# HKUST-Aerial-Robotics/FIESTA

Hardware: NVIDIA H100
Metric: esdf_voxel_updates_per_s (higher is better)
Workload: dtype int32+f64

## Files before the change

### fiesta_b200/csrc/fb_exact.cu

```cuda
#include <cub/cub.cuh>
#include <stdio.h>
#include <stdlib.h>
#include <algorithm>
#include <chrono>
#include "fb_common.cuh"
#include "fb_exact.h"

#define XNONE 0xffffffffu
#define XMB_NONE 0xffffffffffffffffull

__device__ __forceinline__ void x_coords(const FbGeom &g, uint32_t ii, int &x, int &y, int &z) {
  z = ii % (unsigned)g.pz; const unsigned xy = ii / (unsigned)g.pz; y = xy % (unsigned)g.gy; x = xy / (unsigned)g.gy;
}
__device__ __forceinline__ unsigned x_d2(int x, int y, int z, uint32_t c) {
  int ox, oy, oz; fb_unpack(c, ox, oy, oz); ox -= x; oy -= y; oz -= z;
  return (unsigned)(ox * ox + oy * oy + oz * oz);
}
__device__ __forceinline__ unsigned x_dist_of(int x, int y, int z, uint32_t c) { return c < 2u ? 0xffffffffu : x_d2(x, y, z, c); }

__global__ void k_x_flag_exist(const uint32_t *list, unsigned n, const double *occ, double l_occ, uint8_t *flags, int want) {
  const unsigned i = blockIdx.x * blockDim.x + threadIdx.x;
  if (i < n) flags[i] = ((occ[list[i]] > l_occ) ? 1 : 0) == want;
}
__global__ void k_x_apply_seed(FbGeom g, const uint32_t *E, unsigned n, uint32_t *cobs, unsigned long long *LS, unsigned long long t0) {
  const unsigned i = blockIdx.x * blockDim.x + threadIdx.x;
  if (i >= n) return;
  const uint32_t ii = E[i];
  int x, y, z; x_coords(g, ii, x, y, z);
  cobs[ii] = fb_pack(x, y, z);
  LS[ii] = t0 + i;
}

__global__ void k_x_del_minpos(const uint32_t *del, unsigned n, const double *occ, double l_occ, uint32_t *scratch) {
  const unsigned i = blockIdx.x * blockDim.x + threadIdx.x;
  if (i < n && !(occ[del[i]] > l_occ)) atomicMin(&scratch[del[i]], i);
}
__global__ void k_x_del_flag(const uint32_t *del, unsigned n, const double *occ, double l_occ, const uint32_t *scratch, uint8_t *flags) {
  const unsigned i = blockIdx.x * blockDim.x + threadIdx.x;
  if (i < n) flags[i] = (!(occ[del[i]] > l_occ) && scratch[del[i]] == i) ? 1 : 0;
}
__global__ void k_x_del_rank(const uint32_t *sel, unsigned n, uint32_t *scratch) {
  const unsigned i = blockIdx.x * blockDim.x + threadIdx.x;
  if (i < n) scratch[sel[i]] = i;
}
__global__ void k_x_scan_deps(FbGeom g, const uint32_t *cobs, const uint32_t *occbits, const uint32_t *rank, const unsigned long long *LS,
                              unsigned long long *k1, unsigned long long *k2, uint32_t *dv, unsigned *ndep, unsigned cap, int shift) {
  for (long long v = (long long)blockIdx.x * blockDim.x + threadIdx.x; v < g.ptotal; v += (long long)gridDim.x * blockDim.x) {
    const uint32_t c = cobs[v] & FB_CODE_MASK;
    bool dep = false;
    unsigned r = 0;
    if (c >= 2u) {
      int ox, oy, oz; fb_unpack(c, ox, oy, oz);
      const long long oi = fb_ii(g, ox, oy, oz);
      if (!((__ldg(&occbits[oi >> 5]) >> (oi & 31)) & 1u)) { r = rank[oi]; dep = r != XNONE; }
    }
    const unsigned slot = fb_warp_append(ndep, dep);
    if (dep && slot < cap) {
      const unsigned long long inv = ~LS[v];
      if (shift) k1[slot] = ((unsigned long long)r << shift) | (inv & ((1ull << shift) - 1ull));
      else { k1[slot] = r; k2[slot] = inv; }
      dv[slot] = (uint32_t)v;
    }
  }
}
__global__ void k_x_unset(const uint32_t *list, unsigned n, uint32_t *scratch) {
  const unsigned i = blockIdx.x * blockDim.x + threadIdx.x;
  if (i < n) scratch[list[i]] = XNONE;
}
__global__ void k_x_iota(uint32_t *a, unsigned n) { const unsigned i = blockIdx.x * blockDim.x + threadIdx.x; if (i < n) a[i] = i; }
__global__ void k_x_gather64(const unsigned long long *src, const uint32_t *idx, unsigned n, unsigned long long *dst) {
  const unsigned i = blockIdx.x * blockDim.x + threadIdx.x; if (i < n) dst[i] = src[idx[i]];
}
__global__ void k_x_gather32(const uint32_t *src, const uint32_t *idx, unsigned n, uint32_t *dst) {
  const unsigned i = blockIdx.x * blockDim.x + threadIdx.x; if (i < n) dst[i] = src[idx[i]];
}
__global__ void k_x_set_ord(const uint32_t *deps, unsigned n, uint32_t *ord, uint32_t *nc, uint8_t *nk) {
  const unsigned i = blockIdx.x * blockDim.x + threadIdx.x;
  if (i < n) { ord[deps[i]] = i; nc[i] = FB_INF; nk[i] = 24; }
}
__global__ void k_x_fill32(uint32_t *a, size_t n, uint32_t val) {
  for (size_t i = (size_t)blockIdx.x * blockDim.x + threadIdx.x; i < n; i += (size_t)gridDim.x * blockDim.x) a[i] = val;
}
__global__ void k_x_fill64(unsigned long long *a, size_t n, unsigned long long val) {
  for (size_t i = (size_t)blockIdx.x * blockDim.x + threadIdx.x; i < n; i += (size_t)gridDim.x * blockDim.x) a[i] = val;
}

static inline unsigned nblk(size_t n, unsigned t = 256) { return (unsigned)((n + t - 1) / t); }

static int x_select(FbExact *X, const uint32_t *in, const uint8_t *flags, uint32_t *out, unsigned n, unsigned *count, cudaStream_t s) {
  *count = 0;
  if (n == 0) return FIESTA_OK;
  size_t bytes = 0;
  CK(cub::DeviceSelect::Flagged(nullptr, bytes, in, flags, out, X->d_count.p, (int)n, s));
  CK(X->cub_tmp.grow(bytes, s));
  CK(cub::DeviceSelect::Flagged(X->cub_tmp.p, bytes, in, flags, out, X->d_count.p, (int)n, s));
  CK(cudaMemcpyAsync(X->h_count, X->d_count, 4, cudaMemcpyDeviceToHost, s));
  CK(cudaStreamSynchronize(s));
  *count = *X->h_count;
  return FIESTA_OK;
}
static int x_sort_pairs(FbExact *X, const unsigned long long *kin, unsigned long long *kout, const uint32_t *vin, uint32_t *vout, unsigned n, cudaStream_t s,
                        int key_bits = 64) {
  size_t bytes = 0;
  CK(cub::DeviceRadixSort::SortPairs(nullptr, bytes, kin, kout, vin, vout, (int)n, 0, key_bits, s));
  CK(X->cub_tmp.grow(bytes, s));
  CK(cub::DeviceRadixSort::SortPairs(X->cub_tmp.p, bytes, kin, kout, vin, vout, (int)n, 0, key_bits, s));
  return FIESTA_OK;
}
int fb_exact_init(FbExact *X, const FbGeom &g, int device, cudaStream_t s) {
  const size_t P = (size_t)g.ptotal;
  CK(fb_xrelax_init());
  X->relax_blocks = fb_xrelax_blocks(device);
  if (X->relax_blocks <= 0 || X->relax_blocks > FB_X_MAX_BLOCKS) { fb_set_error("exact mode init: k_x_relax does not fit on this device"); return FIESTA_ERR_CUDA; }
  CK(X->MB.alloc(P)); CK(X->LS.alloc(P)); CK(X->tkey.alloc(P));
  CK(X->touched.alloc(P));
  CK(X->SUM.alloc(P)); CK(X->SUMg.alloc(P)); CK(cudaMemsetAsync(X->SUMg, 0, P * 4, s));
  CK(X->emask.alloc(P));
  CK(X->wstamp.alloc(P)); CK(cudaMemsetAsync(X->wstamp, 0, P * 4, s));
  for (int k = 0; k < 3; ++k) { CK(X->W[k].alloc(P)); CK(X->F[k].alloc(P)); CK(cudaMemsetAsync(X->W[k], 0, P * 4, s)); }
  for (int k = 0; k < 2; ++k) CK(X->E[k].alloc(P));
  X->dense_min = 16384u;
  if (const char *e = getenv("FIESTA_X_DENSE")) { long v = atol(e); if (v >= 0 && v <= (1 << 24)) X->dense_min = (unsigned)v; }
  if (const char *e = getenv("FIESTA_X_ASYNC")) X->async = atol(e) != 0;
  if (const char *e = getenv("FIESTA_X_SMALL_ASYNC")) X->small_async = atol(e) != 0;
  X->small_max = FB_X_SMALL_DEFAULT;
  if (const char *e = getenv("FIESTA_X_SMALL")) { long v = atol(e); if (v >= 0 && v <= 65536) X->small_max = (unsigned)v; }
  CK(X->slotc.alloc(((size_t)X->small_max + 1) * 32));
  const size_t c0 = P / 8 > (1u << 20) ? P / 8 : (1u << 20);
  for (FbDevBuf<unsigned long long> *b : {&X->k1, &X->k2, &X->k1b, &X->k2b}) CK(b->grow(c0, s));
  for (FbDevBuf<uint32_t> *b : {&X->dv, &X->idx[0], &X->idx[1], &X->deps, &X->nc[0], &X->nc[1], &X->sel}) CK(b->grow(c0, s));
  CK(X->flags.grow(c0, s)); CK(X->flags2.grow(c0, s));
  CK(X->cub_tmp.grow(c0 * 16 + (64u << 20), s));
  CK(X->d_ctl.alloc(1)); CK(cudaMemsetAsync(X->d_ctl, 0, sizeof(FbXCtl), s));
  CK(X->h_ctl.alloc(1));
  CK(X->d_count.alloc(4)); CK(X->d_flag.alloc(4));
  CK(X->h_count.alloc(4));
  CK(cudaMemsetAsync(X->d_count, 0, 16, s)); CK(cudaMemsetAsync(X->d_flag, 0, 16, s));
  k_x_fill64<<<FB_SMS * 8, 256, 0, s>>>(X->MB, P, XMB_NONE);
  CK(cudaMemsetAsync(X->tkey, 0, P * 8, s));
  CK(cudaMemsetAsync(X->LS, 0, P * 8, s));
  X->tclock = 1; X->key_base = 0; X->key_epoch = 1; X->key_hi = 1ull << FB_KEY_BITS; X->gen_id = 0; X->wclock = 0; X->sclock = 0;
  CK(cudaGetLastError());
  return FIESTA_OK;
}

int fb_exact_queue_crossings(FbExact *X, const unsigned long long *ins_key, const uint32_t *ins_vox, const unsigned long long *del_key,
                             const uint32_t *del_vox, FbDevBuf<uint32_t> &ins, unsigned *n_ins, FbDevBuf<uint32_t> &del, unsigned *n_del,
                             cudaStream_t s, int *launches) {
  int r;
  CK(cudaMemcpyAsync(X->h_count, X->d_count, 8, cudaMemcpyDeviceToHost, s));
  CK(cudaStreamSynchronize(s));
  const unsigned ni = X->h_count[0], nd = X->h_count[1];
  CK(ins.grow((size_t)*n_ins + ni, s, *n_ins));
  CK(del.grow((size_t)*n_del + nd, s, *n_del));
  CK(X->k1b.grow(ni > nd ? ni : nd, s));
  if (ni) { if ((r = x_sort_pairs(X, ins_key, X->k1b, ins_vox, ins + *n_ins, ni, s, FB_KEY_BITS))) return r; *n_ins += ni; *launches += 1; }
  if (nd) { if ((r = x_sort_pairs(X, del_key, X->k1b, del_vox, del + *n_del, nd, s, FB_KEY_BITS))) return r; *n_del += nd; *launches += 1; }
  return FIESTA_OK;
}
int fb_exact_next_epoch(FbExact *X, const FbGeom &g, cudaStream_t s) {
  X->key_base = 0;
  if (++X->key_epoch >= (1u << (64 - FB_KEY_BITS))) {
    CK(cudaMemsetAsync(X->tkey, 0, (size_t)g.ptotal * 8, s));
    X->key_epoch = 1;
  }
  X->key_hi = (unsigned long long)X->key_epoch << FB_KEY_BITS;
  return FIESTA_OK;
}

int fb_exact_update_esdf(FbExact *X, const FbGeom &g, uint32_t *cobs, uint32_t *scratch, const double *occ, const uint32_t *occbits, double l_occ,
                         const uint32_t *ins, unsigned n_ins, const uint32_t *del, unsigned n_del, cudaStream_t s, FbExactStats *st, int *launches) {
  int r;
  const size_t P = (size_t)g.ptotal;
  memset(st, 0, sizeof(*st));
  CK(X->flags.grow((size_t)(n_ins > n_del ? n_ins : n_del) + 16, s));
  static const bool xdbg = getenv("FIESTA_DEBUG_X") != nullptr;
  auto now = [] { return std::chrono::steady_clock::now(); };
  auto ms = [](std::chrono::steady_clock::time_point a, std::chrono::steady_clock::time_point b) { return std::chrono::duration<double, std::milli>(b - a).count(); };
  const auto t_begin = now();
  unsigned nE = 0, ndep_run = 0;
  unsigned long long ls_deps = 0;
  bool scratch_ok = X->scratch_clean;
  if (n_ins) {
    k_x_flag_exist<<<nblk(n_ins), 256, 0, s>>>(ins, n_ins, occ, l_occ, X->flags, 1);
    if ((r = x_select(X, ins, X->flags, X->E[0], n_ins, &nE, s))) return r;
    if (nE) k_x_apply_seed<<<nblk(nE), 256, 0, s>>>(g, X->E[0], nE, cobs, X->LS, X->tclock);
    X->tclock += nE;
    *launches += 2;
  }
  if (n_del) {
    CK(X->sel.grow((size_t)n_del + 16, s));
    if (!X->scratch_clean) { k_x_fill32<<<FB_SMS * 8, 256, 0, s>>>(scratch, P, XNONE); *launches += 1; }
    scratch_ok = true;
    X->scratch_clean = false;
    k_x_del_minpos<<<nblk(n_del), 256, 0, s>>>(del, n_del, occ, l_occ, scratch);
    k_x_del_flag<<<nblk(n_del), 256, 0, s>>>(del, n_del, occ, l_occ, scratch, X->flags);
    unsigned nd = 0;
    if ((r = x_select(X, del, X->flags, X->sel, n_del, &nd, s))) return r;
    k_x_unset<<<nblk(n_del), 256, 0, s>>>(del, n_del, scratch);
    *launches += 3;
    if (nd) {
      k_x_del_rank<<<nblk(nd), 256, 0, s>>>(X->sel, nd, scratch);
      int rank_bits = 1; while ((1ull << rank_bits) < (unsigned long long)nd) ++rank_bits;
      int clock_bits = 1; while (clock_bits < 64 && (X->tclock >> clock_bits)) ++clock_bits;
      const bool two_sorts = getenv("FIESTA_X_TWO_SORTS") != nullptr;
      const int shift = (rank_bits + clock_bits <= 64 && !two_sorts) ? 64 - rank_bits : 0;
      unsigned ndep = 0;
      for (int attempt = 0; attempt < 2; ++attempt) {
        const size_t cap = std::min({X->dv.cap, X->k1.cap, X->k2.cap});
        CK(cudaMemsetAsync(X->d_count, 0, 4, s));
        k_x_scan_deps<<<FB_SMS * 16, 256, 0, s>>>(g, cobs, occbits, scratch, X->LS, X->k1, X->k2, X->dv, X->d_count, (unsigned)cap, shift);
        CK(cudaMemcpyAsync(X->h_count, X->d_count, 4, cudaMemcpyDeviceToHost, s));
        CK(cudaStreamSynchronize(s));
        ndep = *X->h_count;
        *launches += 1;
        if (ndep <= cap) break;
        CK(X->dv.grow(ndep, s));
        CK(X->k1.grow(ndep, s));
        CK(X->k2.grow(ndep, s));
      }
      st->dependants = ndep;
      k_x_unset<<<nblk(nd), 256, 0, s>>>(X->sel, nd, scratch);
      if (ndep) {
        CK(X->k1b.grow(ndep, s));
        CK(X->k2b.grow(ndep, s));
        CK(X->idx[0].grow(ndep, s));
        CK(X->idx[1].grow(ndep, s));
        CK(X->deps.grow(ndep, s));
        CK(X->nc[0].grow(ndep, s));
        CK(X->nc[1].grow(ndep, s));
        CK(X->flags.grow(ndep, s));
        if (shift) {
          if ((r = x_sort_pairs(X, X->k1, X->k1b, X->dv, X->deps, ndep, s))) return r;
          *launches += 1;
        } else {
          k_x_iota<<<nblk(ndep), 256, 0, s>>>(X->idx[0], ndep);
          if ((r = x_sort_pairs(X, X->k2, X->k2b, X->idx[0], X->idx[1], ndep, s))) return r;
          k_x_gather64<<<nblk(ndep), 256, 0, s>>>(X->k1, X->idx[1], ndep, X->k1b);
          if ((r = x_sort_pairs(X, X->k1b, X->k2b, X->idx[1], X->idx[0], ndep, s))) return r;
          k_x_gather32<<<nblk(ndep), 256, 0, s>>>(X->dv, X->idx[0], ndep, X->deps);
          *launches += 5;
        }
        CK(X->flags2.grow(ndep, s));
        k_x_set_ord<<<nblk(ndep), 256, 0, s>>>(X->deps, ndep, scratch, X->nc[0], X->flags2);
        *launches += 1;
        ndep_run = ndep; ls_deps = X->tclock;
        X->tclock += ndep;
      }
    }
  }
  st->generations = 0;
  if (xdbg) { cudaStreamSynchronize(s); fprintf(stderr, "[x] seeds+deletes %.2f ms (reseed rounds %u, dependants %u)\n", ms(t_begin, now()), st->reseed_rounds, st->dependants); }
  if (nE || ndep_run) {
    if (xdbg && !X->d_dbg) CK(X->d_dbg.alloc(FB_X_DBG_WORDS));
    if (xdbg) CK(cudaMemsetAsync(X->d_dbg, 0, FB_X_DBG_WORDS * 8, s));
    if (X->sclock > 0xf0000000u) { CK(cudaMemsetAsync(X->SUMg, 0, P * 4, s)); X->sclock = 0; }
    if (X->gen_id > 0xf0000000u) X->gen_id = 0;
    if (X->wclock > 0xf0000000u) { CK(cudaMemsetAsync(X->wstamp, 0, P * 4, s)); X->wclock = 0; }
    FbXCtl *h = X->h_ctl;
    memset(h, 0, sizeof(*h));
    h->gen_id = X->gen_id; h->wclock = X->wclock; h->tclock = X->tclock; h->sclock = X->sclock;
    CK(cudaMemcpyAsync(X->d_ctl, h, sizeof(FbXCtl), cudaMemcpyHostToDevice, s));
    CK(fb_xrelax_launch(X, g, cobs, nE, X->deps, ndep_run, scratch, X->nc[0], X->flags2, occbits, ls_deps, xdbg ? X->d_dbg.p : nullptr, s));
    if (ndep_run) k_x_unset<<<nblk(ndep_run), 256, 0, s>>>(X->deps, ndep_run, scratch);
    CK(cudaMemcpyAsync(h, X->d_ctl, sizeof(FbXCtl), cudaMemcpyDeviceToHost, s));
    CK(cudaStreamSynchronize(s));
    *launches += 1;
    if (h->err) {
      if (h->err == 3u) {
        for (int k = 0; k < 3; ++k) CK(cudaMemsetAsync(X->W[k], 0, P * 4, s));
        CK(cudaMemsetAsync(X->wstamp, 0, P * 4, s));
        X->wclock = 0;
      }
      fb_set_error(h->err == 1u ? "exact mode: generation with more than 2^27 entries"
                   : h->err == 3u ? "exact mode: a wait of the asynchronous work queue exceeded its bound" : "exact mode: behaviour fixpoint did not converge");
      return FIESTA_ERR_CUDA;
    }
    X->gen_id = h->gen_id; X->wclock = h->wclock; X->tclock = h->tclock; X->sclock = h->sclock;
    st->generations = h->generations; st->reseed_rounds = h->reseed_rounds; st->eval_rounds = h->rounds; st->dense_rounds = h->dense_rounds;
    st->voxels_changed = h->voxels_changed; st->expansions = h->expansions;
    if (xdbg) {
      static unsigned long long hd[FB_X_DBG_WORDS];
      static double cyc_per_us = 0;
      if (cyc_per_us == 0) { int dev = 0, khz = 0; CK(cudaGetDevice(&dev)); CK(cudaDeviceGetAttribute(&khz, cudaDevAttrClockRate, dev)); cyc_per_us = khz / 1000.0; }
      CK(cudaMemcpy(hd, X->d_dbg, sizeof(hd), cudaMemcpyDeviceToHost));
      static const char *cat[20] = {"S", "round1", "rounds", "dense", "commit", "apply", "s.round1", "s.rounds", "s.commit", "s.apply", "top", "empty-barrier",
                                    "reseed.rounds", "reseed.assemble", "", "", "async", "", "refresh", "s.async"};
      fprintf(stderr, "[x] reseed rounds %u; phases (us, count):", st->reseed_rounds);
      for (int c = 0; c < 20; ++c)
        if (*cat[c]) fprintf(stderr, " %s %.0f/%llu", cat[c], hd[FB_XDBG_PHASE + 2 * c] / cyc_per_us, hd[FB_XDBG_PHASE + 2 * c + 1]);
      fprintf(stderr, "\n");
      fprintf(stderr, "[x] round work (summed longest CTA work time us / summed list length):");
      for (int c : {1, 2, 3, 6, 7}) fprintf(stderr, " %s %.0f/%llu", cat[c], hd[FB_XDBG_WORK + 2 * c] / cyc_per_us, hd[FB_XDBG_WORK + 2 * c + 1]);
      fprintf(stderr, "\n");
      for (int h = 0; h < 2; ++h) {
        fprintf(stderr, "[x] list-length histogram %s (log2 bucket=rounds):", h ? "s.rounds" : "rounds");
        for (int b = 0; b < 32; ++b) if (hd[FB_XDBG_NWH + 32 * h + b]) fprintf(stderr, " %d=%llu", b, hd[FB_XDBG_NWH + 32 * h + b]);
        fprintf(stderr, "\n");
      }
      fprintf(stderr, "[x] async: evaluations %llu dirty %llu pushes %llu spin %.0f us\n", hd[FB_XDBG_Q + 0], hd[FB_XDBG_Q + 1], hd[FB_XDBG_Q + 2],
              hd[FB_XDBG_Q + 3] / cyc_per_us);
      for (int gq = 0; gq < 2; ++gq) { fprintf(stderr, "[x] gen %d work lists:", gq); for (int r = 0; r < 512 && hd[FB_XDBG_ROUNDS + gq * 512 + r]; ++r) fprintf(stderr, " %llu", hd[FB_XDBG_ROUNDS + gq * 512 + r]); fprintf(stderr, "\n"); }
      fprintf(stderr, "[x] work-list entries: evaluated %llu refreshed %llu reseeded %llu\n", hd[FB_XDBG_PHASE + 2 * 14], hd[FB_XDBG_PHASE + 2 * 14 + 1], hd[FB_XDBG_PHASE + 2 * 15]);
      fprintf(stderr, "[x] gens %u rounds %u dense %u deps %u nE0 %u |", st->generations, st->eval_rounds, st->dense_rounds, st->dependants, nE);
      for (unsigned q = 0; q < st->generations && q < FB_XDBG_GENS; ++q) fprintf(stderr, " %llu/%llu/%.1fus", hd[3 * q], hd[3 * q + 1], hd[3 * q + 2] / cyc_per_us);
      fprintf(stderr, "\n");
    }
  }
  X->scratch_clean = scratch_ok;
  return FIESTA_OK;
}
```

### fiesta_b200/csrc/fb_exact.h

```cpp
#pragma once
#include "fb_common.cuh"

#define FB_X_MAX_BLOCKS 256
#define FB_X_SMALL_DEFAULT 32768u
#define FB_XDBG_GENS 1024
#define FB_XDBG_NCAT 24
#define FB_XDBG_NQ 8
#define FB_XDBG_PHASE (3 * FB_XDBG_GENS)
#define FB_XDBG_ROUNDS (FB_XDBG_PHASE + 2 * FB_XDBG_NCAT)
#define FB_XDBG_WMAX (FB_XDBG_ROUNDS + 2 * 512)
#define FB_XDBG_WORK (FB_XDBG_WMAX + 4096)
#define FB_XDBG_NWH (FB_XDBG_WORK + 2 * FB_XDBG_NCAT)
#define FB_XDBG_Q (FB_XDBG_NWH + 2 * 32)
#define FB_X_DBG_WORDS (FB_XDBG_Q + FB_XDBG_NQ)

struct FbExactStats {
  unsigned long long expansions;
  unsigned long long voxels_changed;
  unsigned generations, eval_rounds, dense_rounds, reseed_rounds, dependants;
};

struct FbXCtl {
  unsigned bar, err;
  unsigned sclock, pad1;
  unsigned nW[3], nF[3];
  unsigned gen_id, wclock;
  unsigned generations, rounds, dense_rounds, reseed_rounds;
  unsigned long long tclock, expansions, voxels_changed;
  unsigned partial[FB_X_MAX_BLOCKS];
  alignas(128) unsigned long long qtail;
  alignas(128) unsigned qhead;
  alignas(128) unsigned qdone;
};

struct FbExact {
  FbDevBuf<unsigned long long> MB;
  FbDevBuf<unsigned long long> LS;
  FbDevBuf<unsigned long long> tkey;
  FbDevBuf<uint32_t> touched;
  unsigned long long tclock = 0;
  unsigned long long key_base = 0;
  unsigned long long key_hi = 0;
  unsigned key_epoch = 0;
  FbDevBuf<unsigned> d_count, d_flag;
  FbHostBuf<unsigned> h_count;
  bool scratch_clean = false;
  FbDevBuf<uint4> SUM;
  FbDevBuf<uint32_t> SUMg;
  unsigned gen_id = 0, wclock = 0, sclock = 0;
  FbDevBuf<uint32_t> emask;
  FbDevBuf<uint32_t> W[3], F[3];
  FbDevBuf<uint32_t> wstamp;
  FbDevBuf<uint32_t> slotc;
  unsigned dense_min = 0;
  unsigned small_max = 0;
  bool async = true;
  bool small_async = false;
  FbDevBuf<FbXCtl> d_ctl;
  FbHostBuf<FbXCtl> h_ctl;
  FbDevBuf<unsigned long long> d_dbg;
  int relax_blocks = 0;
  FbDevBuf<uint32_t> E[2], sel;
  FbDevBuf<unsigned long long> k1, k2, k1b, k2b;
  FbDevBuf<uint32_t> dv, idx[2], deps, nc[2];
  FbDevBuf<uint8_t> flags, flags2;
  FbDevBuf<char> cub_tmp;
};

int fb_exact_init(FbExact *X, const FbGeom &g, int device, cudaStream_t s);
int fb_exact_queue_crossings(FbExact *X, const unsigned long long *ins_key, const uint32_t *ins_vox, const unsigned long long *del_key,
                             const uint32_t *del_vox, FbDevBuf<uint32_t> &ins, unsigned *n_ins, FbDevBuf<uint32_t> &del, unsigned *n_del,
                             cudaStream_t s, int *launches);
int fb_exact_next_epoch(FbExact *X, const FbGeom &g, cudaStream_t s);
int fb_exact_update_esdf(FbExact *X, const FbGeom &g, uint32_t *cobs, uint32_t *scratch, const double *occ, const uint32_t *occbits, double l_occ,
                         const uint32_t *ins, unsigned n_ins, const uint32_t *del, unsigned n_del, cudaStream_t s, FbExactStats *st, int *launches);
cudaError_t fb_xrelax_init();
int fb_xrelax_blocks(int device);
cudaError_t fb_xrelax_launch(FbExact *X, const FbGeom &g, uint32_t *cobs, unsigned nE0, const uint32_t *deps, unsigned ndep, uint32_t *ord, uint32_t *nc, uint8_t *nk,
                             const uint32_t *occbits, unsigned long long ls_deps, unsigned long long *dbg, cudaStream_t s);
```

### fiesta_b200/csrc/fb_xrelax.cu

```cuda
#include <stdio.h>
#include "fb_common.cuh"
#include "fb_exact.h"
#include "fb_divmagic.h"

#define XT 1024
#define XW (XT / 32)
#define XNONE 0xffffffffu
#define X_DEAD 0ull
#define X_PULL 1ull
#define X_PUSH 2ull
#define XMB_NONE 0xffffffffffffffffull
#define X_NOFF 129
#define X_MAX_ROUNDS 4000000u
#define XGB 8
#define XRC 8
#define XDBG_PHASE FB_XDBG_PHASE
#define XDBG_ROUNDS FB_XDBG_ROUNDS
#define XDBG_WMAX FB_XDBG_WMAX

static __constant__ int x_dirs[24][3] = {
    {-1, 0, 0}, {1, 0, 0}, {0, -1, 0}, {0, 1, 0}, {0, 0, -1}, {0, 0, 1},
    {-1, -1, 0}, {1, 1, 0}, {0, -1, -1}, {0, 1, 1}, {-1, 0, -1}, {1, 0, 1},
    {-1, 1, 0}, {1, -1, 0}, {0, -1, 1}, {0, 1, -1}, {1, 0, -1}, {-1, 0, 1},
    {-2, 0, 0}, {2, 0, 0}, {0, -2, 0}, {0, 2, 0}, {0, 0, -2}, {0, 0, 2}};
static __constant__ int x_off_c[X_NOFF];

__device__ __forceinline__ unsigned x_vi(const FbGeom &g, int x, int y, int z) { return (unsigned)((x * g.gy + y) * g.pz + z); }
__device__ __forceinline__ bool x_in_grid(const FbGeom &g, int x, int y, int z) {
  return (unsigned)x < (unsigned)g.gx && (unsigned)y < (unsigned)g.gy && (unsigned)z < (unsigned)g.gz;
}
__device__ __forceinline__ bool x_in_range(const FbGeom &g, int x, int y, int z) {
  return (unsigned)(x - g.min_vec[0]) <= (unsigned)(g.max_vec[0] - g.min_vec[0]) && (unsigned)(y - g.min_vec[1]) <= (unsigned)(g.max_vec[1] - g.min_vec[1]) &&
         (unsigned)(z - g.min_vec[2]) <= (unsigned)(g.max_vec[2] - g.min_vec[2]);
}
__device__ __forceinline__ int x_dc(int j, int k) {
  const int D[24][3] = {{-1, 0, 0}, {1, 0, 0}, {0, -1, 0}, {0, 1, 0}, {0, 0, -1}, {0, 0, 1}, {-1, -1, 0}, {1, 1, 0}, {0, -1, -1}, {0, 1, 1}, {-1, 0, -1}, {1, 0, 1},
                        {-1, 1, 0}, {1, -1, 0}, {0, -1, 1}, {0, 1, -1}, {1, 0, -1}, {-1, 0, 1}, {-2, 0, 0}, {2, 0, 0}, {0, -2, 0}, {0, 2, 0}, {0, 0, -2}, {0, 0, 2}};
  return D[j][k];
}
__device__ __forceinline__ unsigned long long x_writer_word(const FbGeom &g, const unsigned long long *MB, unsigned v, int x, int y, int z, int j, bool inr) {
  const int dx = x_dc(j, 0), dy = x_dc(j, 1), dz = x_dc(j, 2);
  const bool ok = inr && (dx == 0 || (unsigned)(x - dx) < (unsigned)g.gx) && (dy == 0 || (unsigned)(y - dy) < (unsigned)g.gy) &&
                  (dz == 0 || (unsigned)(z - dz) < (unsigned)g.gz);
  return ok ? __ldcg(&MB[v - (unsigned)((dx * g.gy + dy) * g.pz + dz)]) : XMB_NONE;
}

struct XShared {
  int off[X_NOFF];
  int dir[32];
  unsigned char slot[25 * 24];
  unsigned char self[32];
  unsigned red[XW], red2[XW];
  unsigned base, total;
  unsigned qdone;
};

__device__ __forceinline__ unsigned x_d2(int x, int y, int z, uint32_t c) {
  int ox, oy, oz; fb_unpack(c, ox, oy, oz); ox -= x; oy -= y; oz -= z;
  return (unsigned)(ox * ox + oy * oy + oz * oz);
}
__device__ __forceinline__ unsigned x_dist_of(int x, int y, int z, uint32_t c) { return c < 2u ? 0xffffffffu : x_d2(x, y, z, c); }
__device__ __forceinline__ unsigned long long x_mb(unsigned par, unsigned i, unsigned long long kind, uint32_t code) {
  return ((unsigned long long)(par & 1u) << 63) | ((unsigned long long)i << 33) | (kind << 31) | (unsigned long long)(code & FB_CODE_MASK);
}
__device__ __forceinline__ unsigned x_mb_idx(unsigned long long w) { return (unsigned)(w >> 33) & 0x7ffffffu; }
__device__ __forceinline__ unsigned x_mb_par(unsigned long long w) { return (unsigned)(w >> 63); }
__device__ __forceinline__ unsigned long long x_mb_kind(unsigned long long w) { return (w >> 31) & 3ull; }
__device__ __forceinline__ uint32_t x_mb_code(unsigned long long w) { return (uint32_t)(w & FB_CODE_MASK); }

struct XState { unsigned d; uint32_t c; unsigned ts; };
struct XNb { unsigned long long w[X_NOFF + 3]; uint32_t c[28]; };

template <bool WANT_FIRST>
__device__ __forceinline__ XState x_gather(const FbGeom &g, const uint32_t *cobs, const unsigned long long *MB, int x, int y, int z, unsigned T,
                                           unsigned &first, uint32_t &snap) {
  XState s;
  const unsigned v = x_vi(g, x, y, z);
  const bool inr = x_in_range(g, x, y, z);
  unsigned long long w[XGB];
  const uint32_t snap_raw = __ldcg(&cobs[v]);
  const unsigned long long wown = __ldcg(&MB[v]);
#pragma unroll
  for (int j = 0; j < XGB; ++j) w[j] = x_writer_word(g, MB, v, x, y, z, j, inr);
  snap = snap_raw & FB_CODE_MASK;
  s.c = snap; s.d = (snap_raw & FB_DINF) ? 0xffffffffu : x_dist_of(x, y, z, s.c); s.ts = XNONE;
  first = XNONE;
  const unsigned d0 = s.d;
  if (s.c == FB_UNKNOWN) return s;
#pragma unroll
  for (int h = 0; h < 24 / XGB; ++h) {
    if (h >= 1) {
#pragma unroll
      for (int j = 0; j < XGB; ++j) w[j] = x_writer_word(g, MB, v, x, y, z, XGB * h + j, inr);
    }
#pragma unroll
    for (int j = 0; j < XGB; ++j) {
      const unsigned long long ww = w[j];
      if (ww == XMB_NONE || x_mb_kind(ww) != X_PUSH) continue;
      const unsigned ts = x_mb_idx(ww) * 32u + (unsigned)(XGB * h + j);
      const uint32_t c = x_mb_code(ww);
      const unsigned d = x_d2(x, y, z, c);
      if (d < d0) {
        if (WANT_FIRST && ts < first) first = ts;
        if (ts < T && (d < s.d || (d == s.d && ts < s.ts))) { s.d = d; s.c = c; s.ts = ts; }
      }
    }
  }
  if (wown != XMB_NONE && x_mb_kind(wown) == X_PULL) {
    const unsigned ts = x_mb_idx(wown) * 32u + 24u;
    const uint32_t c = x_mb_code(wown);
    const unsigned d = x_d2(x, y, z, c);
    if (d < d0) {
      if (WANT_FIRST && ts < first) first = ts;
      if (ts < T && (d < s.d || (d == s.d && ts < s.ts))) { s.d = d; s.c = c; s.ts = ts; }
    }
  }
  return s;
}
__device__ __forceinline__ void x_summarize(const FbGeom &g, const uint32_t *cobs, const unsigned long long *MB, uint4 *SUM, int x, int y, int z) {
  unsigned first; uint32_t snap;
  const XState f = x_gather<true>(g, cobs, MB, x, y, z, XNONE, first, snap);
  SUM[x_vi(g, x, y, z)] = make_uint4(first, f.ts, f.c, snap);
}
template <bool USE_SUM>
__device__ __forceinline__ XState x_state(const FbGeom &g, const uint32_t *cobs, const unsigned long long *MB, const uint4 *SUM, int x, int y, int z,
                                          unsigned T, uint32_t &snap) {
  unsigned first;
  if (USE_SUM) {
    const uint4 u = __ldcg(&SUM[x_vi(g, x, y, z)]);
    snap = u.w;
    XState s;
    if (u.x == XNONE || T <= u.x) { s.c = u.w; s.d = x_dist_of(x, y, z, s.c); s.ts = XNONE; return s; }
    if (T > u.y) { s.c = u.z; s.d = x_dist_of(x, y, z, s.c); s.ts = u.y; return s; }
  }
  return x_gather<false>(g, cobs, MB, x, y, z, T, first, snap);
}

__device__ __forceinline__ unsigned x_ld_acquire(const unsigned *p) {
  unsigned v;
  asm volatile("ld.acquire.gpu.global.u32 %0, [%1];" : "=r"(v) : "l"(p) : "memory");
  return v;
}
__device__ __forceinline__ void x_gsync(unsigned *bar, unsigned &target) {
  __syncthreads();
  if (threadIdx.x == 0) {
    target += gridDim.x;
    asm volatile("red.release.gpu.global.add.u32 [%0], %1;" ::"l"(bar), "r"(1u) : "memory");
    while (x_ld_acquire(bar) < target) { }
  }
  __syncthreads();
}

struct XArgs {
  FbGeom g;
  uint32_t *cobs;
  unsigned long long *MB, *LS;
  uint4 *SUM;
  uint32_t *SUMg;
  uint32_t *E[2];
  uint32_t *emask;
  uint32_t *W[3], *F[3];
  uint32_t *wstamp;
  uint32_t *slotc;
  FbXCtl *ctl;
  unsigned nE0, small_max, dense_min;
  const uint32_t *deps; unsigned ndep;
  uint32_t *ord;
  uint32_t *nc;
  uint8_t *nk;
  const uint32_t *occbits;
  unsigned long long ls_deps;
  unsigned long long *dbg;
  unsigned div_pz_m, div_pz_s, div_gy_m, div_gy_s;
  unsigned async_on;
  unsigned small_async_on;
};
__device__ __forceinline__ unsigned x_div(unsigned n, unsigned m, unsigned s) { return m ? (__umulhi(n, m) >> s) : n; }
__device__ __forceinline__ void x_coords(const XArgs &a, uint32_t ii, int &x, int &y, int &z) {
  const unsigned xy = x_div(ii, a.div_pz_m, a.div_pz_s);
  z = (int)(ii - xy * (unsigned)a.g.pz);
  const unsigned xx = x_div(xy, a.div_gy_m, a.div_gy_s);
  y = (int)(xy - xx * (unsigned)a.g.gy);
  x = (int)xx;
}

__device__ __forceinline__ void x_unpack_off(int o, int &dx, int &dy, int &dz) { dx = (o & 15) - 4; dy = ((o >> 4) & 15) - 4; dz = ((o >> 8) & 15) - 4; }

__device__ __forceinline__ void x_claim_summaries(const XArgs &a, const XShared &sh, unsigned lane, int x, int y, int z, unsigned sclock) {
  if (lane >= 25u) return;
  int dx, dy, dz; x_unpack_off(sh.dir[lane], dx, dy, dz);
  const int nx = x + dx, ny = y + dy, nz = z + dz;
  if (!x_in_grid(a.g, nx, ny, nz) || !(lane == 24u || x_in_range(a.g, nx, ny, nz))) return;
  const unsigned n = x_vi(a.g, nx, ny, nz);
  if (__ldcg(&a.SUMg[n]) != sclock && atomicExch(&a.SUMg[n], sclock) != sclock) x_summarize(a.g, a.cobs, a.MB, a.SUM, nx, ny, nz);
}

__device__ __forceinline__ void x_refresh_summaries(const XArgs &a, const XShared &sh, unsigned lane, unsigned i, uint32_t p, int x, int y, int z) {
  unsigned long long w = 0;
  if (lane == 0) w = __ldcg(&a.MB[p]);
  w = __shfl_sync(0xffffffffu, w, 0);
  if (lane >= 25u) return;
  int dx, dy, dz; x_unpack_off(sh.dir[lane], dx, dy, dz);
  const int nx = x + dx, ny = y + dy, nz = z + dz;
  if (!x_in_grid(a.g, nx, ny, nz) || !(lane == 24u || x_in_range(a.g, nx, ny, nz))) return;
  const uint4 u = __ldcg(&a.SUM[x_vi(a.g, nx, ny, nz)]);
  if (u.w == FB_UNKNOWN) return;
  const unsigned ts = i * 32u + lane;
  bool redo = u.x == ts || u.y == ts;
  if (!redo) {
    const unsigned long long kind = x_mb_kind(w);
    const uint32_t c = x_mb_code(w);
    if (((kind == X_PUSH && lane < 24u) || (kind == X_PULL && lane == 24u)) && c >= 2u) {
      const unsigned d = x_d2(nx, ny, nz, c);
      if (u.y == XNONE) redo = true;
      else { const unsigned bd = x_d2(nx, ny, nz, u.z); redo = ts < u.x || d < bd || (d == bd && ts < u.y); }
    }
  }
  if (redo) x_summarize(a.g, a.cobs, a.MB, a.SUM, nx, ny, nz);
}

__device__ __forceinline__ void x_list_affected(const XArgs &a, const XShared &sh, unsigned lane, unsigned i, int x, int y, int z, unsigned nof,
                                                unsigned wclock, unsigned out) {
  const FbGeom &g = a.g;
  unsigned long long w[5];
#pragma unroll
  for (int t = 0; t < 5; ++t) {
    const unsigned o = lane + 32u * (unsigned)t;
    w[t] = XMB_NONE;
    if (o < nof) {
      int dx, dy, dz; x_unpack_off(sh.off[o], dx, dy, dz);
      const int nx = x + dx, ny = y + dy, nz = z + dz;
      if (x_in_grid(g, nx, ny, nz)) w[t] = __ldcg(&a.MB[x_vi(g, nx, ny, nz)]);
    }
  }
  unsigned j[5], st[5];
#pragma unroll
  for (int t = 0; t < 5; ++t) {
    j[t] = w[t] != XMB_NONE ? x_mb_idx(w[t]) : 0u;
    st[t] = (w[t] != XMB_NONE && j[t] > i) ? __ldcg(&a.wstamp[j[t]]) : wclock;
  }
  unsigned pm = 0;
#pragma unroll
  for (int t = 0; t < 5; ++t)
    if (st[t] != wclock && atomicExch(&a.wstamp[j[t]], wclock) != wclock) pm |= 1u << t;
  const unsigned cnt = (unsigned)__popc(pm);
  unsigned incl = cnt;
#pragma unroll
  for (int o = 1; o < 32; o <<= 1) { const unsigned v = __shfl_up_sync(0xffffffffu, incl, o); if ((int)lane >= o) incl += v; }
  const unsigned total = __shfl_sync(0xffffffffu, incl, 31);
  if (total == 0u) return;
  unsigned base = 0;
  if (lane == 0) base = atomicAdd(&a.ctl->nW[out], total);
  base = __shfl_sync(0xffffffffu, base, 0) + incl - cnt;
#pragma unroll
  for (int t = 0; t < 5; ++t) if ((pm >> t) & 1u) a.W[out][base++] = j[t];
}

template <bool USE_SUM>
__device__ __forceinline__ unsigned long long x_eval(const XArgs &a, const XShared &sh, unsigned lane, unsigned par, unsigned i, uint32_t p, int x, int y, int z) {
  const FbGeom &g = a.g;
  const unsigned T0 = i * 32u;
  int qx = x, qy = y, qz = z;
  bool valid = lane == 24;
  if (lane < 24) {
    int dx, dy, dz; x_unpack_off(sh.dir[lane], dx, dy, dz);
    qx += dx; qy += dy; qz += dz;
    valid = x_in_range(g, qx, qy, qz) && x_in_grid(g, qx, qy, qz);
  }
  XState st; st.d = 0xffffffffu; st.c = 0; st.ts = XNONE;
  uint32_t snap = 0;
  if (valid) st = x_state<USE_SUM>(g, a.cobs, a.MB, a.SUM, qx, qy, qz, T0, snap);
  const unsigned sd = __shfl_sync(0xffffffffu, st.d, 24);
  const uint32_t sc = __shfl_sync(0xffffffffu, st.c, 24);
  const uint32_t c0 = __shfl_sync(0xffffffffu, snap, 24);
  if (sd != x_dist_of(x, y, z, c0)) return x_mb(par, i, X_DEAD, 0);
  unsigned long long key = ~0ull;
  if (lane < 24 && valid && st.c >= 2u) {
    const unsigned t = x_d2(x, y, z, st.c);
    if (t < sd) key = ((unsigned long long)t << 8) | lane;
  }
  unsigned long long best = key;
#pragma unroll
  for (int o = 16; o > 0; o >>= 1) { const unsigned long long other = __shfl_xor_sync(0xffffffffu, best, o); best = other < best ? other : best; }
  if (best == ~0ull) return x_mb(par, i, X_PUSH, sc);
  return x_mb(par, i, X_PULL, __shfl_sync(0xffffffffu, st.c, (int)(best & 0xffu)));
}

__device__ __forceinline__ void x_stage(const XArgs &a, const XShared &sh, XNb &nb, unsigned lane, int x, int y, int z) {
  const FbGeom &g = a.g;
  unsigned long long w[5];
#pragma unroll
  for (int t = 0; t < 5; ++t) {
    const unsigned o = lane + 32u * (unsigned)t;
    w[t] = XMB_NONE;
    if (o < X_NOFF) {
      int dx, dy, dz; x_unpack_off(sh.off[o], dx, dy, dz);
      const int nx = x + dx, ny = y + dy, nz = z + dz;
      if (x_in_grid(g, nx, ny, nz)) w[t] = __ldcg(&a.MB[x_vi(g, nx, ny, nz)]);
    }
  }
  uint32_t c = 0;
  if (lane < 25u) {
    int dx, dy, dz; x_unpack_off(sh.dir[lane], dx, dy, dz);
    const int nx = x + dx, ny = y + dy, nz = z + dz;
    if (x_in_grid(g, nx, ny, nz)) c = __ldcg(&a.cobs[x_vi(g, nx, ny, nz)]);
  }
  __syncwarp();
#pragma unroll
  for (int t = 0; t < 5; ++t) { const unsigned o = lane + 32u * (unsigned)t; if (o < X_NOFF) nb.w[o] = w[t]; }
  if (lane < 25u) nb.c[lane] = c;
  __syncwarp();
}
__device__ __forceinline__ XState x_state_nb(const FbGeom &g, const XShared &sh, const XNb &nb, unsigned lane, int qx, int qy, int qz, unsigned T, uint32_t &snap) {
  XState s;
  const uint32_t raw = nb.c[lane];
  snap = raw & FB_CODE_MASK;
  s.c = snap; s.d = (raw & FB_DINF) ? 0xffffffffu : x_dist_of(qx, qy, qz, snap); s.ts = XNONE;
  const unsigned d0 = s.d;
  if (snap == FB_UNKNOWN) return s;
  if (x_in_range(g, qx, qy, qz)) {
#pragma unroll 8
    for (int k = 0; k < 24; ++k) {
      const unsigned long long ww = nb.w[sh.slot[lane * 24u + (unsigned)k]];
      if (ww == XMB_NONE || x_mb_kind(ww) != X_PUSH) continue;
      const unsigned ts = x_mb_idx(ww) * 32u + (unsigned)k;
      const uint32_t c = x_mb_code(ww);
      const unsigned d = x_d2(qx, qy, qz, c);
      if (d < d0 && ts < T && (d < s.d || (d == s.d && ts < s.ts))) { s.d = d; s.c = c; s.ts = ts; }
    }
  }
  const unsigned long long wown = nb.w[sh.self[lane]];
  if (wown != XMB_NONE && x_mb_kind(wown) == X_PULL) {
    const unsigned ts = x_mb_idx(wown) * 32u + 24u;
    const uint32_t c = x_mb_code(wown);
    const unsigned d = x_d2(qx, qy, qz, c);
    if (d < d0 && ts < T && (d < s.d || (d == s.d && ts < s.ts))) { s.d = d; s.c = c; s.ts = ts; }
  }
  return s;
}
__device__ __forceinline__ unsigned long long x_eval_nb(const XArgs &a, const XShared &sh, const XNb &nb, unsigned lane, unsigned par, unsigned i, int x, int y, int z) {
  const FbGeom &g = a.g;
  const unsigned T0 = i * 32u;
  int qx = x, qy = y, qz = z;
  bool valid = lane == 24;
  if (lane < 24) {
    int dx, dy, dz; x_unpack_off(sh.dir[lane], dx, dy, dz);
    qx += dx; qy += dy; qz += dz;
    valid = x_in_range(g, qx, qy, qz) && x_in_grid(g, qx, qy, qz);
  }
  XState st; st.d = 0xffffffffu; st.c = 0; st.ts = XNONE;
  uint32_t snap = 0;
  if (valid) st = x_state_nb(g, sh, nb, lane, qx, qy, qz, T0, snap);
  const unsigned sd = __shfl_sync(0xffffffffu, st.d, 24);
  const uint32_t sc = __shfl_sync(0xffffffffu, st.c, 24);
  const uint32_t c0 = __shfl_sync(0xffffffffu, snap, 24);
  if (sd != x_dist_of(x, y, z, c0)) return x_mb(par, i, X_DEAD, 0);
  unsigned long long key = ~0ull;
  if (lane < 24 && valid && st.c >= 2u) {
    const unsigned t = x_d2(x, y, z, st.c);
    if (t < sd) key = ((unsigned long long)t << 8) | lane;
  }
  unsigned long long best = key;
#pragma unroll
  for (int o = 16; o > 0; o >>= 1) { const unsigned long long other = __shfl_xor_sync(0xffffffffu, best, o); best = other < best ? other : best; }
  if (best == ~0ull) return x_mb(par, i, X_PUSH, sc);
  return x_mb(par, i, X_PULL, __shfl_sync(0xffffffffu, st.c, (int)(best & 0xffu)));
}
__device__ __forceinline__ void x_list_affected_nb(const XArgs &a, const XNb &nb, unsigned lane, unsigned i, unsigned nof, unsigned wclock, unsigned out) {
  unsigned j[5], st[5];
#pragma unroll
  for (int t = 0; t < 5; ++t) {
    const unsigned o = lane + 32u * (unsigned)t;
    const unsigned long long w = o < nof ? nb.w[o] : XMB_NONE;
    j[t] = w != XMB_NONE ? x_mb_idx(w) : 0u;
    st[t] = (w != XMB_NONE && j[t] > i) ? __ldcg(&a.wstamp[j[t]]) : wclock;
  }
  unsigned pm = 0;
#pragma unroll
  for (int t = 0; t < 5; ++t)
    if (st[t] != wclock && atomicExch(&a.wstamp[j[t]], wclock) != wclock) pm |= 1u << t;
  const unsigned cnt = (unsigned)__popc(pm);
  unsigned incl = cnt;
#pragma unroll
  for (int o = 1; o < 32; o <<= 1) { const unsigned v = __shfl_up_sync(0xffffffffu, incl, o); if ((int)lane >= o) incl += v; }
  const unsigned total = __shfl_sync(0xffffffffu, incl, 31);
  if (total == 0u) return;
  unsigned base = 0;
  if (lane == 0) base = atomicAdd(&a.ctl->nW[out], total);
  base = __shfl_sync(0xffffffffu, base, 0) + incl - cnt;
#pragma unroll
  for (int t = 0; t < 5; ++t) if ((pm >> t) & 1u) a.W[out][base++] = j[t];
}

__device__ __forceinline__ unsigned x_block_scan(XShared &sh, unsigned c, unsigned lane, unsigned wid, unsigned &total) {
  unsigned incl = c;
#pragma unroll
  for (int o = 1; o < 32; o <<= 1) { const unsigned t = __shfl_up_sync(0xffffffffu, incl, o); if ((int)lane >= o) incl += t; }
  __syncthreads();
  if (lane == 31) sh.red[wid] = incl;
  __syncthreads();
  const unsigned v = sh.red[lane]; unsigned s = v;
#pragma unroll
  for (int o = 1; o < 32; o <<= 1) { const unsigned t = __shfl_up_sync(0xffffffffu, s, o); if ((int)lane >= o) s += t; }
  total = __shfl_sync(0xffffffffu, s, 31);
  return __shfl_sync(0xffffffffu, s - v, (int)wid) + incl - c;
}

__device__ __forceinline__ unsigned x_warp_append_n(unsigned *counter, unsigned n, unsigned lane) {
  const unsigned act = __activemask(), below = (1u << lane) - 1u;
  unsigned pre = 0, total = 0;
#pragma unroll
  for (int bit = 0; bit < 4; ++bit) {
    const unsigned m = __ballot_sync(act, (n >> bit) & 1u);
    pre += (unsigned)__popc(m & below) << bit;
    total += (unsigned)__popc(m) << bit;
  }
  if (total == 0u) return 0u;
  const int leader = __ffs(act) - 1;
  unsigned base = 0;
  if ((int)lane == leader) base = atomicAdd(counter, total);
  return __shfl_sync(act, base, leader) + pre;
}

#define X_Q_FULL 0x80000000u
#define X_Q_WAIT_NS 2000000000ull
__device__ __forceinline__ unsigned x_ld_relaxed(const unsigned *p) {
  unsigned v;
  asm volatile("ld.relaxed.gpu.global.u32 %0, [%1];" : "=r"(v) : "l"(p) : "memory");
  return v;
}
__device__ __forceinline__ unsigned long long x_globaltimer() {
  unsigned long long t;
  asm volatile("mov.u64 %0, %%globaltimer;" : "=l"(t));
  return t;
}
__device__ __forceinline__ void x_q_abort(const XArgs &a) {
  atomicCAS(&a.ctl->err, 0u, 3u);
  atomicExch(&a.ctl->qdone, 1u);
}
__device__ __forceinline__ unsigned x_q_count(const XArgs &a, XShared &sh, unsigned long long delta) {
  const unsigned long long old = atomicAdd(&a.ctl->qtail, delta);
  if ((unsigned)((old + delta) >> 32) == 0u) { atomicExch(&a.ctl->qdone, 1u); sh.qdone = 1u; }
  return (unsigned)old;
}
__device__ __forceinline__ void x_q_put(const XArgs &a, XShared &sh, uint32_t *ring, unsigned cap, unsigned idx, unsigned e) {
  unsigned *slot = &ring[idx % cap];
  const volatile unsigned *done = &sh.qdone;
  unsigned cur = x_ld_relaxed(slot);
  const unsigned long long t0 = x_globaltimer();
  for (unsigned it = 0;; ++it) {
    if (!(cur & X_Q_FULL)) {
      const unsigned o = atomicCAS(slot, cur, e | X_Q_FULL);
      if (o == cur) return;
      cur = o;
      continue;
    }
    if (*done) return;
    if ((it & 15u) == 15u) {
      if (x_ld_acquire(&a.ctl->qdone)) { sh.qdone = 1u; return; }
      if (x_globaltimer() - t0 > X_Q_WAIT_NS) { x_q_abort(a); sh.qdone = 1u; return; }
    }
    __nanosleep(64);
    cur = x_ld_relaxed(slot);
  }
}
template <bool DBG>
__device__ __forceinline__ unsigned x_q_take(const XArgs &a, XShared &sh, uint32_t *ring, unsigned cap, unsigned &h) {
  if (h == XNONE) h = atomicAdd(&a.ctl->qhead, 1u);
  unsigned *slot = &ring[h % cap];
  const volatile unsigned *done = &sh.qdone;
  const long long c0 = DBG ? clock64() : 0;
  unsigned long long t0 = 0;
  unsigned ns = 32;
  for (unsigned it = 0;; ++it) {
    if (x_ld_relaxed(slot) & X_Q_FULL) {
      const unsigned v = atomicExch(slot, 0u);
      if (v & X_Q_FULL) { h = XNONE; if (DBG) atomicAdd(&a.dbg[FB_XDBG_Q + 3], (unsigned long long)(clock64() - c0)); return v & ~X_Q_FULL; }
    }
    if (*done) break;
    if ((it & 15u) == 15u) {
      if (x_ld_acquire(&a.ctl->qdone)) { sh.qdone = 1u; break; }
      const unsigned long long t = x_globaltimer();
      if (t0 == 0) t0 = t;
      else if (t - t0 > X_Q_WAIT_NS) { x_q_abort(a); sh.qdone = 1u; break; }
    }
    __nanosleep(ns);
    ns = ns < 256u ? 2u * ns : 256u;
  }
  if (DBG) atomicAdd(&a.dbg[FB_XDBG_Q + 3], (unsigned long long)(clock64() - c0));
  return XNONE;
}
__device__ __forceinline__ unsigned x_q_list(const XArgs &a, XShared &sh, const XNb &nb, uint32_t *ring, unsigned cap, unsigned lane, unsigned i, unsigned nof, unsigned A) {
  unsigned j[5], st[5];
#pragma unroll
  for (int t = 0; t < 5; ++t) {
    const unsigned o = lane + 32u * (unsigned)t;
    const unsigned long long w = o < nof ? nb.w[o] : XMB_NONE;
    j[t] = w != XMB_NONE ? x_mb_idx(w) : 0u;
    st[t] = (w != XMB_NONE && j[t] > i) ? x_ld_relaxed(&a.wstamp[j[t]]) : A + 1u;
  }
  unsigned pm = 0;
#pragma unroll
  for (int t = 0; t < 5; ++t)
    if (st[t] != A + 1u && atomicMax(&a.wstamp[j[t]], A + 1u) < A) pm |= 1u << t;
  const unsigned cnt = (unsigned)__popc(pm);
  unsigned incl = cnt;
#pragma unroll
  for (int o = 1; o < 32; o <<= 1) { const unsigned v = __shfl_up_sync(0xffffffffu, incl, o); if ((int)lane >= o) incl += v; }
  const unsigned total = __shfl_sync(0xffffffffu, incl, 31);
  if (total == 0u) return 0u;
  unsigned base = 0;
  if (lane == 0) base = x_q_count(a, sh, (unsigned long long)total * 0x100000001ull);
  base = __shfl_sync(0xffffffffu, base, 0) + incl - cnt;
#pragma unroll
  for (int t = 0; t < 5; ++t) if ((pm >> t) & 1u) x_q_put(a, sh, ring, cap, base++, j[t]);
  return total;
}
template <bool BIG, bool DBG>
__device__ __forceinline__ void x_q_run(const XArgs &a, XShared &sh, XNb &stg, unsigned lane, const uint32_t *E, unsigned nE, uint32_t *ring,
                                        unsigned gen, unsigned A, unsigned fout, unsigned i, bool claimed) {
  const uint32_t p = __ldcg(&E[i]);
  int x, y, z; x_coords(a, p, x, y, z);
  for (;; claimed = false) {
    if (DBG && lane == 0) atomicAdd(&a.dbg[FB_XDBG_Q + 0], 1ull);
    if (!claimed) {
      if (lane == 0) atomicExch(&a.wstamp[i], A);
      __syncwarp();
      __threadfence();
    }
    x_stage(a, sh, stg, lane, x, y, z);
    const unsigned long long old = stg.w[0], nw2 = x_eval_nb(a, sh, stg, lane, gen, i, x, y, z);
    if (nw2 != old) {
      if (lane == 0) {
        a.MB[p] = nw2;
        if (BIG) {
          const unsigned f = atomicAdd(&a.ctl->nF[fout], 1u);
          if (f < (unsigned)a.g.ptotal) a.F[fout][f] = i;
        }
      }
      __syncwarp();
      __threadfence();
      const unsigned np = x_q_list(a, sh, stg, ring, nE, lane, i, (x_mb_kind(old) == X_PUSH || x_mb_kind(nw2) == X_PUSH) ? (unsigned)X_NOFF : 25u, A);
      if (DBG && lane == 0 && np) atomicAdd(&a.dbg[FB_XDBG_Q + 2], (unsigned long long)np);
    }
    unsigned again = 0;
    if (lane == 0) again = atomicCAS(&a.wstamp[i], A, A - 1u) != A ? 1u : 0u;
    if (!__shfl_sync(0xffffffffu, again, 0)) break;
    if (DBG && lane == 0) atomicAdd(&a.dbg[FB_XDBG_Q + 1], 1ull);
  }
}
template <bool DBG>
__device__ void x_async(const XArgs &a, XShared &sh, XNb &stg, unsigned lane, unsigned gwarp, unsigned gwarps, const uint32_t *E, unsigned nE,
                        const uint32_t *wl, unsigned nw, uint32_t *ring, unsigned gen, unsigned A, unsigned fout) {
  for (unsigned q0 = gwarp * 32u; q0 < nw; q0 += gwarps * 32u) {
    const unsigned q = q0 + lane;
    const unsigned e = q < nw ? __ldcg(&wl[q]) : 0u;
    const bool push = q < nw && atomicMax(&a.wstamp[e], A + 1u) < A;
    const unsigned pm = __ballot_sync(0xffffffffu, push), cnt = (unsigned)__popc(pm);
    if (cnt == 0u) continue;
    unsigned base = 0;
    if (lane == 0) base = x_q_count(a, sh, (unsigned long long)cnt * 0x100000001ull);
    base = __shfl_sync(0xffffffffu, base, 0);
    if (push) x_q_put(a, sh, ring, nE, base + (unsigned)__popc(pm & ((1u << lane) - 1u)), e);
    if (DBG && lane == 0) atomicAdd(&a.dbg[FB_XDBG_Q + 2], (unsigned long long)cnt);
  }
  if (lane == 0) x_q_count(a, sh, 0ull - (1ull << 32));
  unsigned h = XNONE;
  for (;;) {
    unsigned i = 0;
    if (lane == 0) i = x_q_take<DBG>(a, sh, ring, nE, h);
    i = __shfl_sync(0xffffffffu, i, 0);
    if (i == XNONE) break;
    x_q_run<true, DBG>(a, sh, stg, lane, E, nE, ring, gen, A, fout, i, false);
    if (lane == 0) x_q_count(a, sh, 0ull - (1ull << 32));
  }
}
template <bool DBG>
__device__ void x_async_small(const XArgs &a, XShared &sh, XNb &stg, unsigned lane, unsigned gwarp, unsigned gwarps, const uint32_t *E, unsigned nE,
                              uint32_t *ring, unsigned gen, unsigned A) {
  const unsigned nwk = min(gwarps, nE);
  if (gwarp >= nwk) return;
  if (gwarp == 0u && lane == 0 && nwk < gwarps) x_q_count(a, sh, 0ull - ((unsigned long long)(gwarps - nwk) << 32));
  for (unsigned s0 = gwarp; s0 < nE; s0 += 32u * nwk) {
    const unsigned e = s0 + lane * nwk;
    unsigned om = __ballot_sync(0xffffffffu, e < nE && atomicMax(&a.wstamp[e], A) < A);
    __threadfence();
    while (om) {
      const unsigned i = s0 + (unsigned)(__ffs(om) - 1) * nwk;
      om &= om - 1u;
      x_q_run<false, DBG>(a, sh, stg, lane, E, nE, ring, gen, A, 0u, i, true);
    }
  }
  if (lane == 0) x_q_count(a, sh, 0ull - (1ull << 32));
  unsigned h = XNONE;
  for (;;) {
    unsigned i = 0;
    if (lane == 0) i = x_q_take<DBG>(a, sh, ring, nE, h);
    i = __shfl_sync(0xffffffffu, i, 0);
    if (i == XNONE) break;
    x_q_run<false, DBG>(a, sh, stg, lane, E, nE, ring, gen, A, 0u, i, false);
    if (lane == 0) x_q_count(a, sh, 0ull - (1ull << 32));
  }
}

__device__ __forceinline__ uint32_t x_reseed_eval(const XArgs &a, unsigned i, int x, int y, int z, unsigned &kc) {
  const FbGeom &g = a.g;
  kc = 24u;
  for (int k = 0; k < 24; ++k) {
    const int nx = x + x_dirs[k][0], ny = y + x_dirs[k][1], nz = z + x_dirs[k][2];
    if (!x_in_range(g, nx, ny, nz) || !x_in_grid(g, nx, ny, nz)) continue;
    const unsigned nv = x_vi(g, nx, ny, nz);
    const unsigned o = __ldcg(&a.ord[nv]);
    uint32_t c;
    if (o != XNONE) { if (o < i) c = __ldcg(&a.nc[o]); else continue; }
    else c = __ldcg(&a.cobs[nv]) & FB_CODE_MASK;
    if (c >= 2u) {
      int ox, oy, oz; fb_unpack(c, ox, oy, oz);
      const unsigned oi = x_vi(g, ox, oy, oz);
      if ((__ldg(&a.occbits[oi >> 5]) >> (oi & 31)) & 1u) { kc = (unsigned)k; return c; }
    }
  }
  return FB_INF;
}

extern __shared__ __align__(16) unsigned char x_dyn_smem[];

template <bool DBG>
__global__ void __launch_bounds__(XT, 1) k_x_relax(const XArgs a) {
  __shared__ XShared sh;
  const FbGeom &g = a.g;
  FbXCtl *ctl = a.ctl;
  const unsigned tid = threadIdx.x, lane = tid & 31u, wid = tid >> 5;
  const unsigned G = gridDim.x, b = blockIdx.x;
  const unsigned gtid = b * XT + tid, gthreads = G * XT;
  const unsigned gwarp = gtid >> 5, gwarps = gthreads >> 5;
  for (unsigned k = tid; k < X_NOFF; k += XT) sh.off[k] = x_off_c[k];
  if (tid < 32) sh.self[tid] = 0;
  if (tid == 0) sh.qdone = 0u;
  if (gtid == 0) a.ctl->qtail = (unsigned long long)gwarps << 32;
  if (tid < 32) sh.dir[tid] = tid < 24 ? ((x_dirs[tid][0] + 4) | ((x_dirs[tid][1] + 4) << 4) | ((x_dirs[tid][2] + 4) << 8)) : (4 | (4 << 4) | (4 << 8));
  __syncthreads();
  for (unsigned q = tid; q < 25u * 24u + 25u; q += XT) {
    const unsigned t = q < 600u ? q / 24u : q - 600u, k = q < 600u ? q % 24u : 24u;
    int tx, ty, tz, kx = 0, ky = 0, kz = 0; x_unpack_off(sh.dir[t], tx, ty, tz);
    if (k < 24u) x_unpack_off(sh.dir[k], kx, ky, kz);
    const int code = (tx - kx + 4) | ((ty - ky + 4) << 4) | ((tz - kz + 4) << 8);
    unsigned found = 0;
    for (unsigned o = 0; o < X_NOFF; ++o) if (sh.off[o] == code) found = o;
    if (q < 600u) sh.slot[q] = (unsigned char)found; else sh.self[t] = (unsigned char)found;
  }
  __syncthreads();
  XNb &stg = reinterpret_cast<XNb *>(x_dyn_smem)[wid];

  unsigned nE = a.nE0, bar_target = 0;
  int cur = 0;
  unsigned gen = ctl->gen_id, wclock = ctl->wclock;
  unsigned long long tclock = ctl->tclock;
  unsigned generations = 0, rounds_total = 0, dense_total = 0;
  unsigned long long changed_total = 0;
  if (DBG) {
    const long long t0 = clock64();
    for (int q = 0; q < 32; ++q) x_gsync(&ctl->bar, bar_target);
    if (gtid == 0) a.dbg[XDBG_PHASE + 2 * 11] = (unsigned long long)(clock64() - t0) / 32ull;
  }
  long long t_ph = DBG ? clock64() : 0;
#define X_LAP(cat) do { if (DBG && gtid == 0) { const long long t_now = clock64(); a.dbg[XDBG_PHASE + 2 * (cat)] += (unsigned long long)(t_now - t_ph); a.dbg[XDBG_PHASE + 2 * (cat) + 1] += 1ull; t_ph = t_now; } } while (0)
  unsigned reseed_rounds = 0;
  if (a.ndep) {
    for (unsigned r = 1;; ++r) {
      const unsigned in = r % 3u, out = (r + 1u) % 3u, zz = (r + 2u) % 3u;
      const unsigned nw = r == 1u ? a.ndep : __ldcg(&ctl->nW[in]);
      if (gtid == 0) ctl->nW[zz] = 0;
      if (r > 1u && nw == 0u) break;
      if (DBG && gtid == 0) a.dbg[XDBG_PHASE + 2 * 15] += nw;
      ++reseed_rounds; ++wclock;
      if (nw <= 2u * gwarps) {
        for (unsigned q = gwarp; q < nw; q += gwarps) {
          const unsigned i = r == 1u ? q : __ldcg(&a.W[in][q]);
          int x, y, z; x_coords(a, __ldcg(&a.deps[i]), x, y, z);
          int dx = 0, dy = 0, dz = 0;
          if (lane < 24u) x_unpack_off(sh.dir[lane], dx, dy, dz);
          const int nx = x + dx, ny = y + dy, nz = z + dz;
          const bool ing = lane < 24u && x_in_grid(g, nx, ny, nz);
          const unsigned nv = ing ? x_vi(g, nx, ny, nz) : 0u;
          const unsigned o = ing ? __ldcg(&a.ord[nv]) : XNONE;
          uint32_t c = 0;
          if (ing && x_in_range(g, nx, ny, nz)) {
            if (o != XNONE) { if (o < i) c = __ldcg(&a.nc[o]); }
            else c = __ldcg(&a.cobs[nv]) & FB_CODE_MASK;
          }
          bool ok = false;
          if (c >= 2u) { int px, py, pz; fb_unpack(c, px, py, pz); const unsigned oi = x_vi(g, px, py, pz); ok = (__ldg(&a.occbits[oi >> 5]) >> (oi & 31)) & 1u; }
          const unsigned vm = __ballot_sync(0xffffffffu, ok);
          const unsigned kc = vm ? (unsigned)(__ffs(vm) - 1) : 24u;
          const uint32_t res = vm ? __shfl_sync(0xffffffffu, c, (int)kc) : FB_INF;
          uint32_t was = 0;
          if (lane == 0) { was = __ldcg(&a.nc[i]); a.nk[i] = (uint8_t)kc; }
          was = __shfl_sync(0xffffffffu, was, 0);
          if (res == was) continue;
          if (lane == 0) a.nc[i] = res;
          bool push = ing && o != XNONE && o > i;
          if (push) {
            const unsigned so = __ldcg(&a.wstamp[o]);
            push = so != wclock;
            if (push && r > 1u && so != wclock - 1u) {
              const unsigned ko = __ldcg(&a.nk[o]), kd = lane ^ 1u;
              push = kd == ko || (kd < ko && res >= 2u);
            }
            push = push && atomicExch(&a.wstamp[o], wclock) != wclock;
          }
          const unsigned slot2 = fb_warp_append(&ctl->nW[out], push);
          if (push) a.W[out][slot2] = o;
        }
      } else
      for (unsigned q = gtid; q < nw; q += gthreads) {
        const unsigned i = r == 1u ? q : __ldcg(&a.W[in][q]);
        int x, y, z; x_coords(a, __ldcg(&a.deps[i]), x, y, z);
        unsigned kc;
        const uint32_t res = x_reseed_eval(a, i, x, y, z, kc);
        const uint32_t was = __ldcg(&a.nc[i]);
        a.nk[i] = (uint8_t)kc;
        if (res == was) continue;
        a.nc[i] = res;
#pragma unroll
        for (int k0 = 0; k0 < 24; k0 += XRC) {
          unsigned o[XRC], so[XRC], ko[XRC];
#pragma unroll
          for (int t = 0; t < XRC; ++t) {
            const int k = k0 + t, nx = x + x_dc(k, 0), ny = y + x_dc(k, 1), nz = z + x_dc(k, 2);
            o[t] = x_in_grid(g, nx, ny, nz) ? __ldcg(&a.ord[x_vi(g, nx, ny, nz)]) : XNONE;
          }
#pragma unroll
          for (int t = 0; t < XRC; ++t) so[t] = (o[t] != XNONE && o[t] > i) ? __ldcg(&a.wstamp[o[t]]) : wclock;
#pragma unroll
          for (int t = 0; t < XRC; ++t) ko[t] = (so[t] != wclock && r > 1u && so[t] != wclock - 1u) ? __ldcg(&a.nk[o[t]]) : XNONE;
          unsigned pm = 0;
#pragma unroll
          for (int t = 0; t < XRC; ++t) {
            const unsigned kd = (unsigned)(k0 + t) ^ 1u;
            bool push = so[t] != wclock;
            if (push && ko[t] != XNONE) push = kd == ko[t] || (kd < ko[t] && res >= 2u);
            if (push && atomicExch(&a.wstamp[o[t]], wclock) != wclock) pm |= 1u << t;
          }
          unsigned slot2 = x_warp_append_n(&ctl->nW[out], (unsigned)__popc(pm), lane);
#pragma unroll
          for (int t = 0; t < XRC; ++t) if ((pm >> t) & 1u) a.W[out][slot2++] = o[t];
        }
      }
      x_gsync(&ctl->bar, bar_target);
    }
    X_LAP(12);
    const unsigned per = (a.ndep + G - 1u) / G;
    const unsigned lo = min(a.ndep, b * per), hi = min(a.ndep, lo + per);
    unsigned mine = 0;
    for (unsigned i = lo + tid; i < hi; i += XT) mine += __ldcg(&a.nc[i]) >= 2u ? 1u : 0u;
    unsigned tot;
    x_block_scan(sh, mine, lane, wid, tot);
    if (tid == 0) ctl->partial[b] = tot;
    if (gtid == 0) { ctl->nW[0] = ctl->nW[1] = ctl->nW[2] = 0; }
    x_gsync(&ctl->bar, bar_target);
    if (wid == 0) {
      unsigned before = 0, all = 0;
      for (unsigned k = lane; k < G; k += 32u) { const unsigned c = __ldcg(&ctl->partial[k]); all += c; if (k < b) before += c; }
#pragma unroll
      for (int o = 16; o > 0; o >>= 1) { before += __shfl_xor_sync(0xffffffffu, before, o); all += __shfl_xor_sync(0xffffffffu, all, o); }
      if (lane == 0) { sh.base = before; sh.total = all; }
    }
    __syncthreads();
    unsigned run = nE + sh.base;
    for (unsigned i0 = lo; i0 < hi; i0 += XT) {
      const unsigned i = i0 + tid;
      uint32_t c = FB_INF, v = 0;
      if (i < hi) {
        c = __ldcg(&a.nc[i]); v = __ldcg(&a.deps[i]);
        a.cobs[v] = c;
        a.LS[v] = a.ls_deps + i;
      }
      unsigned ctot;
      const unsigned pos = x_block_scan(sh, (i < hi && c >= 2u) ? 1u : 0u, lane, wid, ctot);
      if (i < hi && c >= 2u) a.E[0][run + pos] = v;
      run += ctot;
    }
    nE += sh.total;
    x_gsync(&ctl->bar, bar_target);
    X_LAP(13);
  }
  bool big = nE > a.small_max;

  ++gen;
  unsigned sclock = ctl->sclock;
  for (unsigned i = gtid; i < nE; i += gthreads) {
    const uint32_t v = __ldcg(&a.E[0][i]);
    a.MB[v] = x_mb(gen, i, X_PUSH, __ldcg(&a.cobs[v]) & FB_CODE_MASK);
  }
  x_gsync(&ctl->bar, bar_target);

  while (nE) {
    const long long t_gen = DBG ? clock64() : 0;
    X_LAP(10);
    ++generations;
    const uint32_t *E = a.E[cur];
    unsigned rounds = 0;
    bool aborted = false;
    if (big) {
      ++sclock;
      for (unsigned i = gwarp; i < nE; i += gwarps) { int x, y, z; x_coords(a, __ldcg(&E[i]), x, y, z); x_claim_summaries(a, sh, lane, x, y, z, sclock); }
      x_gsync(&ctl->bar, bar_target);
      X_LAP(0);
    }
    for (unsigned r = 1;; ++r) {
      const unsigned in = r % 3u, out = (r + 1u) % 3u, zz = (r + 2u) % 3u;
      const unsigned nw = r == 1u ? nE : __ldcg(&ctl->nW[in]);
      const unsigned nf = (big && r > 1u) ? __ldcg(&ctl->nF[in]) : 0u;
      if (gtid == 0) { ctl->nW[zz] = 0; ctl->nF[zz] = 0; }
      if (r > 1u && nw == 0u && nf == 0u) break;
      if (r > X_MAX_ROUNDS) { if (gtid == 0) ctl->err = 2u; break; }
      if (DBG && gtid == 0) { a.dbg[XDBG_PHASE + 2 * 14] += nw; a.dbg[XDBG_PHASE + 2 * 14 + 1] += nf; }
      if (a.async_on && (big ? r > 1u && nw <= a.dense_min : r == 1u && a.small_async_on)) {
        ++rounds; wclock += 3u;
        const unsigned A = wclock - 1u;
        if (big) x_async<DBG>(a, sh, stg, lane, gwarp, gwarps, E, nE, a.W[in], nw, a.W[out], gen, A, out);
        else x_async_small<DBG>(a, sh, stg, lane, gwarp, gwarps, E, nE, a.W[out], gen, A);
        x_gsync(&ctl->bar, bar_target);
        X_LAP(big ? 16 : 19);
        if (tid == 0) sh.qdone = 0u;
        if (gtid == 0) { ctl->qtail = (unsigned long long)gwarps << 32; ctl->qhead = 0u; ctl->qdone = 0u; }
        if (__ldcg(&ctl->err)) { aborted = true; break; }
        if (!big) break;
        const unsigned nfa = __ldcg(&ctl->nF[out]);
        if (nfa > (unsigned)g.ptotal) {
          ++sclock;
          for (unsigned i = gwarp; i < nE; i += gwarps) { int x, y, z; x_coords(a, __ldcg(&E[i]), x, y, z); x_claim_summaries(a, sh, lane, x, y, z, sclock); }
        } else {
          for (unsigned q = gwarp; q < nf + nfa; q += gwarps) {
            const unsigned i = q < nf ? __ldcg(&a.F[in][q]) : __ldcg(&a.F[out][q - nf]);
            const uint32_t p = __ldcg(&E[i]);
            int x, y, z; x_coords(a, p, x, y, z);
            x_refresh_summaries(a, sh, lane, i, p, x, y, z);
          }
        }
        x_gsync(&ctl->bar, bar_target);
        X_LAP(18);
        break;
      }
      ++rounds; ++wclock;
      const bool dense = big && r > 1u && nw > a.dense_min;
      if (dense) {
        ++dense_total;
        if (nf < nE / 4u) {
          for (unsigned q = gwarp; q < nf; q += gwarps) {
            const unsigned i = __ldcg(&a.F[in][q]);
            const uint32_t p = __ldcg(&E[i]);
            int x, y, z; x_coords(a, p, x, y, z);
            x_refresh_summaries(a, sh, lane, i, p, x, y, z);
          }
        } else {
          ++sclock;
          for (unsigned i = gwarp; i < nE; i += gwarps) { int x, y, z; x_coords(a, __ldcg(&E[i]), x, y, z); x_claim_summaries(a, sh, lane, x, y, z, sclock); }
        }
        x_gsync(&ctl->bar, bar_target);
      }
      const bool use_sum = big && (r == 1u || dense);
      const unsigned nref = (big && !dense) ? nf : 0u;
      const uint32_t *wl = a.W[in];
      const long long t_w0 = DBG ? clock64() : 0;
      for (unsigned q = gwarp; q < nw + nref; q += gwarps) {
        if (q >= nw) {
          const unsigned i = __ldcg(&a.F[in][q - nw]);
          const uint32_t p = __ldcg(&E[i]);
          int x, y, z; x_coords(a, p, x, y, z);
          x_refresh_summaries(a, sh, lane, i, p, x, y, z);
          continue;
        }
        const unsigned i = r == 1u ? q : __ldcg(&wl[q]);
        const uint32_t p = __ldcg(&E[i]);
        int x, y, z; x_coords(a, p, x, y, z);
        if (!use_sum) {
          x_stage(a, sh, stg, lane, x, y, z);
          const unsigned long long old = stg.w[0], nw2 = x_eval_nb(a, sh, stg, lane, gen, i, x, y, z);
          if (nw2 == old) continue;
          if (lane == 0) {
            a.MB[p] = nw2;
            if (big) a.F[out][atomicAdd(&ctl->nF[out], 1u)] = i;
          }
          x_list_affected_nb(a, stg, lane, i, (x_mb_kind(old) == X_PUSH || x_mb_kind(nw2) == X_PUSH) ? (unsigned)X_NOFF : 25u, wclock, out);
          continue;
        }
        unsigned long long old = 0;
        if (lane == 0) old = __ldcg(&a.MB[p]);
        const unsigned long long nb = x_eval<true>(a, sh, lane, gen, i, p, x, y, z);
        old = __shfl_sync(0xffffffffu, old, 0);
        if (nb == old) continue;
        if (lane == 0) {
          a.MB[p] = nb;
          if (big) a.F[out][atomicAdd(&ctl->nF[out], 1u)] = i;
        }
        x_list_affected(a, sh, lane, i, x, y, z, (x_mb_kind(old) == X_PUSH || x_mb_kind(nb) == X_PUSH) ? (unsigned)X_NOFF : 25u, wclock, out);
      }
      if (DBG) { __syncthreads(); if (tid == 0) atomicMax(&a.dbg[XDBG_WMAX + ((rounds_total + rounds) & 4095u)], (unsigned long long)(clock64() - t_w0)); }
      x_gsync(&ctl->bar, bar_target);
      X_LAP(big ? (r == 1u ? 1 : (dense ? 3 : 2)) : (r == 1u ? 6 : 7));
      if (DBG && gtid == 0) {
        if (generations <= 2u && rounds <= 512u) a.dbg[XDBG_ROUNDS + (generations - 1u) * 512u + (rounds - 1u)] = nw;
        const unsigned cat = big ? (r == 1u ? 1u : (dense ? 3u : 2u)) : (r == 1u ? 6u : 7u);
        unsigned long long *wm = &a.dbg[XDBG_WMAX + ((rounds_total + rounds) & 4095u)];
        a.dbg[FB_XDBG_WORK + 2 * cat] += __ldcg(wm); a.dbg[FB_XDBG_WORK + 2 * cat + 1] += nw; *wm = 0;
        if (cat == 2u || cat == 7u) a.dbg[FB_XDBG_NWH + (cat == 7u ? 32u : 0u) + (nw ? 32u - __clz(nw) : 0u)] += 1ull;
      }
    }
    rounds_total += rounds;
    if (rounds > X_MAX_ROUNDS || aborted) break;

    const unsigned per = (nE + G - 1u) / G;
    const unsigned lo = min(nE, b * per), hi = min(nE, lo + per);
    unsigned wcount = 0, wlive = 0;
    for (unsigned i = lo + wid; i < hi; i += XW) {
      const uint32_t p = __ldcg(&E[i]);
      int x, y, z; x_coords(a, p, x, y, z);
      unsigned long long w = 0;
      if (!big) { x_stage(a, sh, stg, lane, x, y, z); w = stg.w[0]; }
      else { if (lane == 0) w = __ldcg(&a.MB[p]); w = __shfl_sync(0xffffffffu, w, 0); }
      const unsigned long long kind = x_mb_kind(w);
      bool win = false;
      if ((kind == X_PUSH && lane < 24) || (kind == X_PULL && lane == 24)) {
        int dx, dy, dz; x_unpack_off(sh.dir[lane], dx, dy, dz);
        const int nx = x + dx, ny = y + dy, nz = z + dz;
        if (x_in_grid(g, nx, ny, nz) && (lane == 24 || x_in_range(g, nx, ny, nz))) {
          const unsigned ts = i * 32u + lane;
          if (big) win = __ldcg(&a.SUM[x_vi(g, nx, ny, nz)]).y == ts;
          else {
            uint32_t snap;
            const XState f = x_state_nb(g, sh, stg, lane, nx, ny, nz, XNONE, snap);
            win = f.ts == ts;
            if (win) a.slotc[ts] = f.c;
          }
        }
      }
      const unsigned m = __ballot_sync(0xffffffffu, win);
      if (lane == 0) { a.emask[i] = m; wcount += __popc(m); wlive += kind != X_DEAD ? 1u : 0u; }
    }
    if (lane == 0) { sh.red[wid] = wcount; sh.red2[wid] = wlive; }
    __syncthreads();
    if (wid == 0) {
      unsigned c = sh.red[lane], l = sh.red2[lane];
#pragma unroll
      for (int o = 16; o > 0; o >>= 1) { c += __shfl_xor_sync(0xffffffffu, c, o); l += __shfl_xor_sync(0xffffffffu, l, o); }
      if (lane == 0) { ctl->partial[b] = c; if (l) atomicAdd(&ctl->expansions, (unsigned long long)l); }
    }
    if (gtid == 0) { ctl->nW[0] = ctl->nW[1] = ctl->nW[2] = 0; ctl->nF[0] = ctl->nF[1] = ctl->nF[2] = 0; }
    x_gsync(&ctl->bar, bar_target);
    X_LAP(big ? 4 : 8);

    if (wid == 0) {
      unsigned before = 0, all = 0;
      for (unsigned k = lane; k < G; k += 32u) { const unsigned c = __ldcg(&ctl->partial[k]); all += c; if (k < b) before += c; }
#pragma unroll
      for (int o = 16; o > 0; o >>= 1) { before += __shfl_xor_sync(0xffffffffu, before, o); all += __shfl_xor_sync(0xffffffffu, all, o); }
      if (lane == 0) { sh.base = before; sh.total = all; }
    }
    __syncthreads();
    const unsigned n2 = sh.total;
    const bool big2 = n2 > a.small_max;
    uint32_t *En = a.E[cur ^ 1];
    unsigned run = sh.base;
    for (unsigned i0 = lo; i0 < hi; i0 += XT) {
      const unsigned i = i0 + tid;
      const uint32_t m = i < hi ? __ldcg(&a.emask[i]) : 0u;
      if (i < hi) {
        const uint32_t p = __ldcg(&E[i]);
        const unsigned long long w = __ldcg(&a.MB[p]);
        if (w != XMB_NONE && x_mb_par(w) == (gen & 1u)) atomicCAS(&a.MB[p], w, XMB_NONE);
      }
      unsigned ctot;
      unsigned r = run + x_block_scan(sh, (unsigned)__popc(m), lane, wid, ctot);
      if (m) {
        const uint32_t p = __ldcg(&E[i]);
        int x, y, z; x_coords(a, p, x, y, z);
        uint32_t me = m;
        while (me) {
          const int k = __ffs(me) - 1; me &= me - 1u;
          int dx, dy, dz; x_unpack_off(sh.dir[k], dx, dy, dz);
          const uint32_t v = (uint32_t)x_vi(g, x + dx, y + dy, z + dz);
          const unsigned ts = i * 32u + (unsigned)k;
          const uint32_t code = big ? __ldcg(&a.SUM[v]).z : __ldcg(&a.slotc[ts]);
          a.cobs[v] = code;
          a.LS[v] = tclock + ts;
          En[r] = v;
          a.MB[v] = x_mb(gen + 1u, r, X_PUSH, code);
          ++r;
        }
      }
      run += ctot;
    }
    if (DBG && gtid == 0 && generations <= FB_XDBG_GENS) { a.dbg[3 * (generations - 1u)] = nE; a.dbg[3 * (generations - 1u) + 1] = rounds; a.dbg[3 * (generations - 1u) + 2] = (unsigned long long)(clock64() - t_gen); }
    tclock += (unsigned long long)nE * 32ull + 1ull;
    changed_total += n2;
    if (n2 >= (1u << 27)) { if (gtid == 0) ctl->err = 1u; break; }
    const bool was_big = big;
    nE = n2; cur ^= 1; big = big2; ++gen;
    x_gsync(&ctl->bar, bar_target);
    X_LAP(was_big ? 5 : 9);
  }
  if (gtid == 0) {
    ctl->gen_id = gen; ctl->wclock = wclock; ctl->tclock = tclock; ctl->sclock = sclock;
    ctl->generations = generations; ctl->reseed_rounds = reseed_rounds; ctl->rounds = rounds_total; ctl->dense_rounds = dense_total; ctl->voxels_changed = changed_total;
  }
}

static bool g_off_ready = false;
cudaError_t fb_xrelax_init() {
  if (g_off_ready) return cudaSuccess;
  static const int D[24][3] = {
      {-1, 0, 0}, {1, 0, 0}, {0, -1, 0}, {0, 1, 0}, {0, 0, -1}, {0, 0, 1},
      {-1, -1, 0}, {1, 1, 0}, {0, -1, -1}, {0, 1, 1}, {-1, 0, -1}, {1, 0, 1},
      {-1, 1, 0}, {1, -1, 0}, {0, -1, 1}, {0, 1, -1}, {1, 0, -1}, {-1, 0, 1},
      {-2, 0, 0}, {2, 0, 0}, {0, -2, 0}, {0, 2, 0}, {0, 0, -2}, {0, 0, 2}};
  int off[1024], n = 0;
  for (int p = -1; p < 24; ++p)
    for (int q = -1; q < 24; ++q) {
      int o[3];
      for (int k = 0; k < 3; ++k) o[k] = (p < 0 ? 0 : D[p][k]) + (q < 0 ? 0 : D[q][k]);
      const int code = (o[0] + 4) | ((o[1] + 4) << 4) | ((o[2] + 4) << 8);
      bool dup = false;
      for (int j = 0; j < n; ++j) dup = dup || off[j] == code;
      if (!dup) off[n++] = code;
    }
  if (n != X_NOFF) return cudaErrorUnknown;
  cudaError_t e = cudaMemcpyToSymbol(x_off_c, off, sizeof(int) * X_NOFF);
  if (e == cudaSuccess) g_off_ready = true;
  return e;
}

int fb_xrelax_blocks(int device) {
  int per_sm = 0, sms = 0;
  for (const void *k : {(const void *)k_x_relax<false>, (const void *)k_x_relax<true>})
    if (cudaOccupancyMaxActiveBlocksPerMultiprocessor(&per_sm, k, XT, sizeof(XNb) * XW) != cudaSuccess || per_sm < 1) return -1;
  if (cudaDeviceGetAttribute(&sms, cudaDevAttrMultiProcessorCount, device) != cudaSuccess) return -1;
  return sms;
}

cudaError_t fb_xrelax_launch(FbExact *X, const FbGeom &g, uint32_t *cobs, unsigned nE0, const uint32_t *deps, unsigned ndep, uint32_t *ord, uint32_t *nc, uint8_t *nk,
                             const uint32_t *occbits, unsigned long long ls_deps, unsigned long long *dbg, cudaStream_t s) {
  XArgs a;
  a.deps = deps; a.ndep = ndep; a.ord = ord; a.nc = nc; a.nk = nk; a.occbits = occbits; a.ls_deps = ls_deps;
  fb_div_make((unsigned)g.pz, a.div_pz_m, a.div_pz_s);
  fb_div_make((unsigned)g.gy, a.div_gy_m, a.div_gy_s);
  a.g = g;
  if (a.g.max_vec[0] < a.g.min_vec[0] || a.g.max_vec[1] < a.g.min_vec[1] || a.g.max_vec[2] < a.g.min_vec[2])
    for (int k = 0; k < 3; ++k) a.g.min_vec[k] = a.g.max_vec[k] = 0x3fffffff;
  a.cobs = cobs; a.MB = X->MB; a.LS = X->LS; a.SUM = X->SUM; a.SUMg = X->SUMg;
  a.E[0] = X->E[0]; a.E[1] = X->E[1]; a.emask = X->emask;
  for (int k = 0; k < 3; ++k) { a.W[k] = X->W[k]; a.F[k] = X->F[k]; }
  a.wstamp = X->wstamp; a.slotc = X->slotc; a.ctl = X->d_ctl; a.nE0 = nE0; a.small_max = X->small_max; a.dense_min = X->dense_min; a.dbg = dbg;
  a.async_on = X->async ? 1u : 0u;
  a.small_async_on = X->small_async ? 1u : 0u;
  void *args[] = {(void *)&a};
  return cudaLaunchCooperativeKernel(dbg ? (void *)k_x_relax<true> : (void *)k_x_relax<false>, dim3(X->relax_blocks), dim3(XT), args, sizeof(XNb) * XW, s);
}
```

Before: 129.9 million.

## Replace iterative reseed fixpoint with classify-closure-resolve reseed kernel

Result: faster. 140.2 million (median of 6 runs) (+7.9%).

```diff
diff --git a/fiesta_b200/csrc/fb_exact.cu b/fiesta_b200/csrc/fb_exact.cu
--- a/fiesta_b200/csrc/fb_exact.cu
+++ b/fiesta_b200/csrc/fb_exact.cu
@@ -74,9 +74,9 @@
 __global__ void k_x_gather32(const uint32_t *src, const uint32_t *idx, unsigned n, uint32_t *dst) {
   const unsigned i = blockIdx.x * blockDim.x + threadIdx.x; if (i < n) dst[i] = src[idx[i]];
 }
-__global__ void k_x_set_ord(const uint32_t *deps, unsigned n, uint32_t *ord, uint32_t *nc, uint8_t *nk) {
-  const unsigned i = blockIdx.x * blockDim.x + threadIdx.x;
-  if (i < n) { ord[deps[i]] = i; nc[i] = FB_INF; nk[i] = 24; }
+__global__ void k_x_set_ord(const uint32_t *deps, unsigned n, uint32_t *ord) {
+  const unsigned i = blockIdx.x * blockDim.x + threadIdx.x;
+  if (i < n) ord[deps[i]] = i;
 }
 __global__ void k_x_fill32(uint32_t *a, size_t n, uint32_t val) {
   for (size_t i = (size_t)blockIdx.x * blockDim.x + threadIdx.x; i < n; i += (size_t)gridDim.x * blockDim.x) a[i] = val;
@@ -129,7 +129,7 @@
   const size_t c0 = P / 8 > (1u << 20) ? P / 8 : (1u << 20);
   for (FbDevBuf<unsigned long long> *b : {&X->k1, &X->k2, &X->k1b, &X->k2b}) CK(b->grow(c0, s));
   for (FbDevBuf<uint32_t> *b : {&X->dv, &X->idx[0], &X->idx[1], &X->deps, &X->nc[0], &X->nc[1], &X->sel}) CK(b->grow(c0, s));
-  CK(X->flags.grow(c0, s)); CK(X->flags2.grow(c0, s));
+  CK(X->flags.grow(c0, s));
   CK(X->cub_tmp.grow(c0 * 16 + (64u << 20), s));
   CK(X->d_ctl.alloc(1)); CK(cudaMemsetAsync(X->d_ctl, 0, sizeof(FbXCtl), s));
   CK(X->h_ctl.alloc(1));
@@ -241,8 +241,7 @@
           k_x_gather32<<<nblk(ndep), 256, 0, s>>>(X->dv, X->idx[0], ndep, X->deps);
           *launches += 5;
         }
-        CK(X->flags2.grow(ndep, s));
-        k_x_set_ord<<<nblk(ndep), 256, 0, s>>>(X->deps, ndep, scratch, X->nc[0], X->flags2);
+        k_x_set_ord<<<nblk(ndep), 256, 0, s>>>(X->deps, ndep, scratch);
         *launches += 1;
         ndep_run = ndep; ls_deps = X->tclock;
         X->tclock += ndep;
@@ -250,7 +249,7 @@
     }
   }
   st->generations = 0;
-  if (xdbg) { cudaStreamSynchronize(s); fprintf(stderr, "[x] seeds+deletes %.2f ms (reseed rounds %u, dependants %u)\n", ms(t_begin, now()), st->reseed_rounds, st->dependants); }
+  if (xdbg) { cudaStreamSynchronize(s); fprintf(stderr, "[x] seeds+deletes %.2f ms (dependants %u)\n", ms(t_begin, now()), st->dependants); }
   if (nE || ndep_run) {
     if (xdbg && !X->d_dbg) CK(X->d_dbg.alloc(FB_X_DBG_WORDS));
     if (xdbg) CK(cudaMemsetAsync(X->d_dbg, 0, FB_X_DBG_WORDS * 8, s));
@@ -259,13 +258,13 @@
     if (X->wclock > 0xf0000000u) { CK(cudaMemsetAsync(X->wstamp, 0, P * 4, s)); X->wclock = 0; }
     FbXCtl *h = X->h_ctl;
     memset(h, 0, sizeof(*h));
-    h->gen_id = X->gen_id; h->wclock = X->wclock; h->tclock = X->tclock; h->sclock = X->sclock;
+    h->gen_id = X->gen_id; h->wclock = X->wclock; h->tclock = X->tclock; h->sclock = X->sclock; h->nE0 = nE;
     CK(cudaMemcpyAsync(X->d_ctl, h, sizeof(FbXCtl), cudaMemcpyHostToDevice, s));
-    CK(fb_xrelax_launch(X, g, cobs, nE, X->deps, ndep_run, scratch, X->nc[0], X->flags2, occbits, ls_deps, xdbg ? X->d_dbg.p : nullptr, s));
+    CK(fb_xrelax_launch(X, g, cobs, X->deps, ndep_run, scratch, X->nc[0], X->nc[1], occbits, ls_deps, xdbg ? X->d_dbg.p : nullptr, s));
     if (ndep_run) k_x_unset<<<nblk(ndep_run), 256, 0, s>>>(X->deps, ndep_run, scratch);
     CK(cudaMemcpyAsync(h, X->d_ctl, sizeof(FbXCtl), cudaMemcpyDeviceToHost, s));
     CK(cudaStreamSynchronize(s));
-    *launches += 1;
+    *launches += ndep_run ? 2 : 1;
     if (h->err) {
       if (h->err == 3u) {
         for (int k = 0; k < 3; ++k) CK(cudaMemsetAsync(X->W[k], 0, P * 4, s));
@@ -284,10 +283,11 @@
       static double cyc_per_us = 0;
       if (cyc_per_us == 0) { int dev = 0, khz = 0; CK(cudaGetDevice(&dev)); CK(cudaDeviceGetAttribute(&khz, cudaDevAttrClockRate, dev)); cyc_per_us = khz / 1000.0; }
       CK(cudaMemcpy(hd, X->d_dbg, sizeof(hd), cudaMemcpyDeviceToHost));
-      static const char *cat[20] = {"S", "round1", "rounds", "dense", "commit", "apply", "s.round1", "s.rounds", "s.commit", "s.apply", "top", "empty-barrier",
-                                    "reseed.rounds", "reseed.assemble", "", "", "async", "", "refresh", "s.async"};
+      static const char *cat[FB_XDBG_NCAT] = {"S", "round1", "rounds", "dense", "commit", "apply", "s.round1", "s.rounds", "s.commit", "s.apply", "top",
+                                              "empty-barrier", "reseed.classify", "reseed.assemble", "", "", "async", "", "refresh", "s.async",
+                                              "reseed.closure", "reseed.choose", "reseed.resolve", ""};
       fprintf(stderr, "[x] reseed rounds %u; phases (us, count):", st->reseed_rounds);
-      for (int c = 0; c < 20; ++c)
+      for (int c = 0; c < FB_XDBG_NCAT; ++c)
         if (*cat[c]) fprintf(stderr, " %s %.0f/%llu", cat[c], hd[FB_XDBG_PHASE + 2 * c] / cyc_per_us, hd[FB_XDBG_PHASE + 2 * c + 1]);
       fprintf(stderr, "\n");
       fprintf(stderr, "[x] round work (summed longest CTA work time us / summed list length):");
@@ -301,7 +301,9 @@
       fprintf(stderr, "[x] async: evaluations %llu dirty %llu pushes %llu spin %.0f us\n", hd[FB_XDBG_Q + 0], hd[FB_XDBG_Q + 1], hd[FB_XDBG_Q + 2],
               hd[FB_XDBG_Q + 3] / cyc_per_us);
       for (int gq = 0; gq < 2; ++gq) { fprintf(stderr, "[x] gen %d work lists:", gq); for (int r = 0; r < 512 && hd[FB_XDBG_ROUNDS + gq * 512 + r]; ++r) fprintf(stderr, " %llu", hd[FB_XDBG_ROUNDS + gq * 512 + r]); fprintf(stderr, "\n"); }
-      fprintf(stderr, "[x] work-list entries: evaluated %llu refreshed %llu reseeded %llu\n", hd[FB_XDBG_PHASE + 2 * 14], hd[FB_XDBG_PHASE + 2 * 14 + 1], hd[FB_XDBG_PHASE + 2 * 15]);
+      fprintf(stderr, "[x] work-list entries: evaluated %llu refreshed %llu\n", hd[FB_XDBG_PHASE + 2 * 14], hd[FB_XDBG_PHASE + 2 * 14 + 1]);
+      fprintf(stderr, "[x] reseed: dependants %u final after classify %llu closure rounds %llu list entries %llu resolve passes %llu\n", st->dependants,
+              hd[FB_XDBG_PHASE + 2 * 15], hd[FB_XDBG_PHASE + 2 * 20 + 1], hd[FB_XDBG_PHASE + 2 * 15 + 1], hd[FB_XDBG_PHASE + 2 * 22 + 1]);
       fprintf(stderr, "[x] gens %u rounds %u dense %u deps %u nE0 %u |", st->generations, st->eval_rounds, st->dense_rounds, st->dependants, nE);
       for (unsigned q = 0; q < st->generations && q < FB_XDBG_GENS; ++q) fprintf(stderr, " %llu/%llu/%.1fus", hd[3 * q], hd[3 * q + 1], hd[3 * q + 2] / cyc_per_us);
       fprintf(stderr, "\n");
diff --git a/fiesta_b200/csrc/fb_exact.h b/fiesta_b200/csrc/fb_exact.h
--- a/fiesta_b200/csrc/fb_exact.h
+++ b/fiesta_b200/csrc/fb_exact.h
@@ -17,12 +17,15 @@
 struct FbExactStats {
   unsigned long long expansions;
   unsigned long long voxels_changed;
-  unsigned generations, eval_rounds, dense_rounds, reseed_rounds, dependants;
+  unsigned generations, eval_rounds, dense_rounds, dependants;
+  unsigned reseed_rounds;
 };
 
 struct FbXCtl {
   unsigned bar, err;
-  unsigned sclock, pad1;
+  unsigned sclock;
+  unsigned rbar;
+  unsigned nE0;
   unsigned nW[3], nF[3];
   unsigned gen_id, wclock;
   unsigned generations, rounds, dense_rounds, reseed_rounds;
@@ -63,7 +66,7 @@
   FbDevBuf<uint32_t> E[2], sel;
   FbDevBuf<unsigned long long> k1, k2, k1b, k2b;
   FbDevBuf<uint32_t> dv, idx[2], deps, nc[2];
-  FbDevBuf<uint8_t> flags, flags2;
+  FbDevBuf<uint8_t> flags;
   FbDevBuf<char> cub_tmp;
 };
 
@@ -76,5 +79,5 @@
                          const uint32_t *ins, unsigned n_ins, const uint32_t *del, unsigned n_del, cudaStream_t s, FbExactStats *st, int *launches);
 cudaError_t fb_xrelax_init();
 int fb_xrelax_blocks(int device);
-cudaError_t fb_xrelax_launch(FbExact *X, const FbGeom &g, uint32_t *cobs, unsigned nE0, const uint32_t *deps, unsigned ndep, uint32_t *ord, uint32_t *nc, uint8_t *nk,
+cudaError_t fb_xrelax_launch(FbExact *X, const FbGeom &g, uint32_t *cobs, const uint32_t *deps, unsigned ndep, uint32_t *ord, uint32_t *nc, uint32_t *M,
                              const uint32_t *occbits, unsigned long long ls_deps, unsigned long long *dbg, cudaStream_t s);
diff --git a/fiesta_b200/csrc/fb_xrelax.cu b/fiesta_b200/csrc/fb_xrelax.cu
--- a/fiesta_b200/csrc/fb_xrelax.cu
+++ b/fiesta_b200/csrc/fb_xrelax.cu
@@ -13,7 +13,6 @@
 #define X_NOFF 129
 #define X_MAX_ROUNDS 4000000u
 #define XGB 8
-#define XRC 8
 #define XDBG_PHASE FB_XDBG_PHASE
 #define XDBG_ROUNDS FB_XDBG_ROUNDS
 #define XDBG_WMAX FB_XDBG_WMAX
@@ -163,11 +162,11 @@
   uint32_t *wstamp;
   uint32_t *slotc;
   FbXCtl *ctl;
-  unsigned nE0, small_max, dense_min;
+  unsigned small_max, dense_min;
   const uint32_t *deps; unsigned ndep;
   uint32_t *ord;
   uint32_t *nc;
-  uint8_t *nk;
+  uint32_t *M;
   const uint32_t *occbits;
   unsigned long long ls_deps;
   unsigned long long *dbg;
@@ -406,22 +405,6 @@
   return __shfl_sync(0xffffffffu, s - v, (int)wid) + incl - c;
 }
 
-__device__ __forceinline__ unsigned x_warp_append_n(unsigned *counter, unsigned n, unsigned lane) {
-  const unsigned act = __activemask(), below = (1u << lane) - 1u;
-  unsigned pre = 0, total = 0;
-#pragma unroll
-  for (int bit = 0; bit < 4; ++bit) {
-    const unsigned m = __ballot_sync(act, (n >> bit) & 1u);
-    pre += (unsigned)__popc(m & below) << bit;
-    total += (unsigned)__popc(m) << bit;
-  }
-  if (total == 0u) return 0u;
-  const int leader = __ffs(act) - 1;
-  unsigned base = 0;
-  if ((int)lane == leader) base = atomicAdd(counter, total);
-  return __shfl_sync(act, base, leader) + pre;
-}
-
 #define X_Q_FULL 0x80000000u
 #define X_Q_WAIT_NS 2000000000ull
 __device__ __forceinline__ unsigned x_ld_relaxed(const unsigned *p) {
@@ -603,27 +586,214 @@
   }
 }
 
-__device__ __forceinline__ uint32_t x_reseed_eval(const XArgs &a, unsigned i, int x, int y, int z, unsigned &kc) {
-  const FbGeom &g = a.g;
-  kc = 24u;
-  for (int k = 0; k < 24; ++k) {
-    const int nx = x + x_dirs[k][0], ny = y + x_dirs[k][1], nz = z + x_dirs[k][2];
-    if (!x_in_range(g, nx, ny, nz) || !x_in_grid(g, nx, ny, nz)) continue;
-    const unsigned nv = x_vi(g, nx, ny, nz);
-    const unsigned o = __ldcg(&a.ord[nv]);
-    uint32_t c;
-    if (o != XNONE) { if (o < i) c = __ldcg(&a.nc[o]); else continue; }
-    else c = __ldcg(&a.cobs[nv]) & FB_CODE_MASK;
-    if (c >= 2u) {
-      int ox, oy, oz; fb_unpack(c, ox, oy, oz);
-      const unsigned oi = x_vi(g, ox, oy, oz);
-      if ((__ldg(&a.occbits[oi >> 5]) >> (oi & 31)) & 1u) { kc = (unsigned)k; return c; }
-    }
-  }
-  return FB_INF;
-}
-
 extern __shared__ __align__(16) unsigned char x_dyn_smem[];
+
+#define X_STATIC 0x20000000u
+#define X_VALID 0x40000000u
+#define X_PAR 0x80000000u
+#define X_LAP(cat) do { if (DBG && gtid == 0) { const long long t_now = clock64(); a.dbg[XDBG_PHASE + 2 * (cat)] += (unsigned long long)(t_now - t_ph); a.dbg[XDBG_PHASE + 2 * (cat) + 1] += 1ull; t_ph = t_now; } } while (0)
+
+template <int K0>
+__device__ __forceinline__ void x_dep_nb(const XArgs &a, int x, int y, int z, unsigned want, unsigned (&nv)[8], unsigned (&o)[8]) {
+#pragma unroll
+  for (int t = 0; t < 8; ++t) {
+    const int nx = x + x_dc(K0 + t, 0), ny = y + x_dc(K0 + t, 1), nz = z + x_dc(K0 + t, 2);
+    nv[t] = ((want >> (K0 + t)) & 1u) && x_in_grid(a.g, nx, ny, nz) && x_in_range(a.g, nx, ny, nz) ? x_vi(a.g, nx, ny, nz) : XNONE;
+    o[t] = nv[t] != XNONE ? __ldcg(&a.ord[nv[t]]) : XNONE;
+  }
+}
+template <int K0>
+__device__ __forceinline__ unsigned x_first_valid(const XArgs &a, int x, int y, int z, unsigned mask, unsigned &par) {
+  unsigned nv[8], o[8], m[8];
+  x_dep_nb<K0>(a, x, y, z, mask, nv, o);
+#pragma unroll
+  for (int t = 0; t < 8; ++t) m[t] = o[t] != XNONE ? __ldcg(&a.M[o[t]]) : 0u;
+#pragma unroll
+  for (int t = 0; t < 8; ++t) if (m[t] & X_VALID) { par = o[t]; return (unsigned)(K0 + t); }
+  return 24u;
+}
+template <int K0>
+__device__ __forceinline__ void x_classify(const XArgs &a, unsigned i, int x, int y, int z, unsigned &mask, uint32_t &sc, bool &done) {
+  unsigned nv[8], o[8];
+  uint32_t c[8];
+  x_dep_nb<K0>(a, x, y, z, 0xffffffu, nv, o);
+#pragma unroll
+  for (int t = 0; t < 8; ++t) c[t] = (nv[t] != XNONE && o[t] == XNONE) ? __ldcg(&a.cobs[nv[t]]) & FB_CODE_MASK : 0u;
+  unsigned e[8];
+#pragma unroll
+  for (int t = 0; t < 8; ++t) {
+    e[t] = 0u;
+    if (c[t] >= 2u) { int ox, oy, oz; fb_unpack(c[t], ox, oy, oz); const unsigned oi = x_vi(a.g, ox, oy, oz); e[t] = (__ldg(&a.occbits[oi >> 5]) >> (oi & 31)) & 1u; }
+  }
+#pragma unroll
+  for (int t = 0; t < 8; ++t) {
+    if (done || nv[t] == XNONE) continue;
+    if (o[t] != XNONE) { if (o[t] < i) mask |= 1u << (K0 + t); }
+    else if (e[t]) { sc = c[t]; done = true; }
+  }
+}
+template <int K0>
+__device__ __forceinline__ void x_mark_later(const XArgs &a, bool act, unsigned o, int x, int y, int z, unsigned out) {
+  unsigned j[8], m[8];
+#pragma unroll
+  for (int t = 0; t < 8; ++t) {
+    const int nx = x + x_dc(K0 + t, 0), ny = y + x_dc(K0 + t, 1), nz = z + x_dc(K0 + t, 2);
+    j[t] = act && x_in_grid(a.g, nx, ny, nz) ? __ldcg(&a.ord[x_vi(a.g, nx, ny, nz)]) : XNONE;
+  }
+#pragma unroll
+  for (int t = 0; t < 8; ++t) m[t] = (j[t] != XNONE && j[t] > o) ? __ldcg(&a.M[j[t]]) : X_VALID;
+#pragma unroll
+  for (int t = 0; t < 8; ++t) {
+    const bool push = !(m[t] & (X_STATIC | X_VALID)) && !(atomicOr(&a.M[j[t]], X_VALID) & X_VALID);
+    const unsigned slot = fb_warp_append(&a.ctl->nW[out], push);
+    if (push) a.W[out][slot] = j[t];
+  }
+}
+
+template <bool DBG>
+__global__ void __launch_bounds__(XT, 1) k_x_reseed(const XArgs a) {
+  __shared__ XShared sh;
+  FbXCtl *ctl = a.ctl;
+  const unsigned tid = threadIdx.x, lane = tid & 31u, wid = tid >> 5, G = gridDim.x, b = blockIdx.x;
+  const unsigned gtid = b * XT + tid, gthreads = G * XT;
+  unsigned bar_target = 0;
+  long long t_ph = DBG ? clock64() : 0;
+  for (unsigned i0 = 0; i0 < a.ndep; i0 += gthreads) {
+    const unsigned i = i0 + gtid;
+    unsigned mask = 0;
+    uint32_t sc = FB_INF;
+    bool done = true;
+    if (i < a.ndep) {
+      int x, y, z; x_coords(a, __ldcg(&a.deps[i]), x, y, z);
+      done = false;
+      x_classify<0>(a, i, x, y, z, mask, sc, done);
+      if (!done) x_classify<8>(a, i, x, y, z, mask, sc, done);
+      if (!done) x_classify<16>(a, i, x, y, z, mask, sc, done);
+      a.nc[i] = sc;
+      a.M[i] = mask | (done ? X_STATIC | X_VALID : 0u);
+    }
+    const bool pull = !done && mask;
+    const unsigned slot = fb_warp_append(&ctl->nW[1], pull);
+    if (pull) a.W[1][slot] = i;
+    if (DBG) { const unsigned f = __popc(__ballot_sync(0xffffffffu, i < a.ndep && !mask)); if ((threadIdx.x & 31u) == 0 && f) atomicAdd(&a.dbg[XDBG_PHASE + 2 * 15], (unsigned long long)f); }
+  }
+  x_gsync(&ctl->rbar, bar_target);
+  X_LAP(12);
+  unsigned r = 1, rounds = 0;
+  for (;; ++r) {
+    const unsigned in = r % 3u, out = (r + 1u) % 3u, zz = (r + 2u) % 3u;
+    const unsigned nw = __ldcg(&ctl->nW[in]);
+    if (gtid == 0) ctl->nW[zz] = 0;
+    if (nw == 0u) break;
+    ++rounds;
+    if (DBG && gtid == 0) a.dbg[XDBG_PHASE + 2 * 15 + 1] += nw;
+    for (unsigned q0 = 0; q0 < nw; q0 += gthreads) {
+      const unsigned q = q0 + gtid;
+      const bool act = q < nw;
+      const unsigned i = act ? __ldcg(&a.W[in][q]) : 0u;
+      int x = 0, y = 0, z = 0;
+      if (act) x_coords(a, __ldcg(&a.deps[i]), x, y, z);
+      if (r == 1u) {
+        unsigned k = 24u, par;
+        if (act) {
+          const unsigned mask = __ldcg(&a.M[i]);
+          k = x_first_valid<0>(a, x, y, z, mask, par);
+          if (k == 24u) k = x_first_valid<8>(a, x, y, z, mask, par);
+          if (k == 24u) k = x_first_valid<16>(a, x, y, z, mask, par);
+          if (k != 24u) a.M[i] = mask | X_VALID;
+        }
+        const unsigned slot = fb_warp_append(&ctl->nW[out], k != 24u);
+        if (k != 24u) a.W[out][slot] = i;
+      } else {
+        const bool push = act && x_in_range(a.g, x, y, z);
+        x_mark_later<0>(a, push, i, x, y, z, out);
+        x_mark_later<8>(a, push, i, x, y, z, out);
+        x_mark_later<16>(a, push, i, x, y, z, out);
+      }
+    }
+    x_gsync(&ctl->rbar, bar_target);
+    X_LAP(20);
+  }
+  {
+    const unsigned out = (r + 1u) % 3u;
+    for (unsigned i0 = 0; i0 < a.ndep; i0 += gthreads) {
+      const unsigned i = i0 + gtid;
+      const unsigned m = i < a.ndep ? __ldcg(&a.M[i]) : 0u;
+      unsigned k = 24u, par = 0;
+      if ((m & X_VALID) && (m & 0xffffffu)) {
+        int x, y, z; x_coords(a, __ldcg(&a.deps[i]), x, y, z);
+        k = x_first_valid<0>(a, x, y, z, m, par);
+        if (k == 24u) k = x_first_valid<8>(a, x, y, z, m, par);
+        if (k == 24u) k = x_first_valid<16>(a, x, y, z, m, par);
+        if (k != 24u) a.nc[i] = X_PAR | par;
+      }
+      const unsigned slot = fb_warp_append(&ctl->nW[out], k != 24u);
+      if (k != 24u) a.W[out][slot] = i;
+    }
+    x_gsync(&ctl->rbar, bar_target);
+    X_LAP(21);
+  }
+  unsigned passes = 0;
+  for (++r;; ++r) {
+    const unsigned in = r % 3u, out = (r + 1u) % 3u, zz = (r + 2u) % 3u;
+    const unsigned nw = __ldcg(&ctl->nW[in]);
+    if (gtid == 0) ctl->nW[zz] = 0;
+    if (nw == 0u) break;
+    ++passes;
+    for (unsigned q0 = 0; q0 < nw; q0 += gthreads) {
+      const unsigned q = q0 + gtid;
+      bool again = false;
+      unsigned i = 0;
+      if (q < nw) {
+        i = __ldcg(&a.W[in][q]);
+        const uint32_t c = __ldcg(&a.nc[__ldcg(&a.nc[i]) & ~X_PAR]);
+        a.nc[i] = c;
+        again = (c & X_PAR) != 0u;
+      }
+      const unsigned slot = fb_warp_append(&ctl->nW[out], again);
+      if (again) a.W[out][slot] = i;
+    }
+    x_gsync(&ctl->rbar, bar_target);
+    X_LAP(22);
+  }
+  const unsigned per = (a.ndep + G - 1u) / G;
+  const unsigned lo = min(a.ndep, b * per), hi = min(a.ndep, lo + per);
+  unsigned mine = 0;
+  for (unsigned i = lo + tid; i < hi; i += XT) mine += __ldcg(&a.nc[i]) >= 2u ? 1u : 0u;
+  unsigned tot;
+  x_block_scan(sh, mine, lane, wid, tot);
+  if (tid == 0) ctl->partial[b] = tot;
+  const unsigned nE = __ldcg(&ctl->nE0);
+  x_gsync(&ctl->rbar, bar_target);
+  if (wid == 0) {
+    unsigned before = 0, all = 0;
+    for (unsigned k = lane; k < G; k += 32u) { const unsigned c = __ldcg(&ctl->partial[k]); all += c; if (k < b) before += c; }
+#pragma unroll
+    for (int o = 16; o > 0; o >>= 1) { before += __shfl_xor_sync(0xffffffffu, before, o); all += __shfl_xor_sync(0xffffffffu, all, o); }
+    if (lane == 0) { sh.base = before; sh.total = all; }
+  }
+  __syncthreads();
+  unsigned run = nE + sh.base;
+  for (unsigned i0 = lo; i0 < hi; i0 += XT) {
+    const unsigned i = i0 + tid;
+    uint32_t c = FB_INF, v = 0;
+    if (i < hi) {
+      c = __ldcg(&a.nc[i]); v = __ldcg(&a.deps[i]);
+      a.cobs[v] = c;
+      a.LS[v] = a.ls_deps + i;
+    }
+    unsigned ctot;
+    const unsigned pos = x_block_scan(sh, (i < hi && c >= 2u) ? 1u : 0u, lane, wid, ctot);
+    if (i < hi && c >= 2u) a.E[0][run + pos] = v;
+    run += ctot;
+  }
+  if (gtid == 0) {
+    ctl->nE0 = nE + sh.total;
+    ctl->reseed_rounds = rounds + passes;
+    ctl->nW[0] = ctl->nW[1] = ctl->nW[2] = 0;
+  }
+  X_LAP(13);
+}
 
 template <bool DBG>
 __global__ void __launch_bounds__(XT, 1) k_x_relax(const XArgs a) {
@@ -652,7 +822,7 @@
   __syncthreads();
   XNb &stg = reinterpret_cast<XNb *>(x_dyn_smem)[wid];
 
-  unsigned nE = a.nE0, bar_target = 0;
+  unsigned nE = ctl->nE0, bar_target = 0;
   int cur = 0;
   unsigned gen = ctl->gen_id, wclock = ctl->wclock;
   unsigned long long tclock = ctl->tclock;
@@ -664,127 +834,6 @@
     if (gtid == 0) a.dbg[XDBG_PHASE + 2 * 11] = (unsigned long long)(clock64() - t0) / 32ull;
   }
   long long t_ph = DBG ? clock64() : 0;
-#define X_LAP(cat) do { if (DBG && gtid == 0) { const long long t_now = clock64(); a.dbg[XDBG_PHASE + 2 * (cat)] += (unsigned long long)(t_now - t_ph); a.dbg[XDBG_PHASE + 2 * (cat) + 1] += 1ull; t_ph = t_now; } } while (0)
-  unsigned reseed_rounds = 0;
-  if (a.ndep) {
-    for (unsigned r = 1;; ++r) {
-      const unsigned in = r % 3u, out = (r + 1u) % 3u, zz = (r + 2u) % 3u;
-      const unsigned nw = r == 1u ? a.ndep : __ldcg(&ctl->nW[in]);
-      if (gtid == 0) ctl->nW[zz] = 0;
-      if (r > 1u && nw == 0u) break;
-      if (DBG && gtid == 0) a.dbg[XDBG_PHASE + 2 * 15] += nw;
-      ++reseed_rounds; ++wclock;
-      if (nw <= 2u * gwarps) {
-        for (unsigned q = gwarp; q < nw; q += gwarps) {
-          const unsigned i = r == 1u ? q : __ldcg(&a.W[in][q]);
-          int x, y, z; x_coords(a, __ldcg(&a.deps[i]), x, y, z);
-          int dx = 0, dy = 0, dz = 0;
-          if (lane < 24u) x_unpack_off(sh.dir[lane], dx, dy, dz);
-          const int nx = x + dx, ny = y + dy, nz = z + dz;
-          const bool ing = lane < 24u && x_in_grid(g, nx, ny, nz);
-          const unsigned nv = ing ? x_vi(g, nx, ny, nz) : 0u;
-          const unsigned o = ing ? __ldcg(&a.ord[nv]) : XNONE;
-          uint32_t c = 0;
-          if (ing && x_in_range(g, nx, ny, nz)) {
-            if (o != XNONE) { if (o < i) c = __ldcg(&a.nc[o]); }
-            else c = __ldcg(&a.cobs[nv]) & FB_CODE_MASK;
-          }
-          bool ok = false;
-          if (c >= 2u) { int px, py, pz; fb_unpack(c, px, py, pz); const unsigned oi = x_vi(g, px, py, pz); ok = (__ldg(&a.occbits[oi >> 5]) >> (oi & 31)) & 1u; }
-          const unsigned vm = __ballot_sync(0xffffffffu, ok);
-          const unsigned kc = vm ? (unsigned)(__ffs(vm) - 1) : 24u;
-          const uint32_t res = vm ? __shfl_sync(0xffffffffu, c, (int)kc) : FB_INF;
-          uint32_t was = 0;
-          if (lane == 0) { was = __ldcg(&a.nc[i]); a.nk[i] = (uint8_t)kc; }
-          was = __shfl_sync(0xffffffffu, was, 0);
-          if (res == was) continue;
-          if (lane == 0) a.nc[i] = res;
-          bool push = ing && o != XNONE && o > i;
-          if (push) {
-            const unsigned so = __ldcg(&a.wstamp[o]);
-            push = so != wclock;
-            if (push && r > 1u && so != wclock - 1u) {
-              const unsigned ko = __ldcg(&a.nk[o]), kd = lane ^ 1u;
-              push = kd == ko || (kd < ko && res >= 2u);
-            }
-            push = push && atomicExch(&a.wstamp[o], wclock) != wclock;
-          }
-          const unsigned slot2 = fb_warp_append(&ctl->nW[out], push);
-          if (push) a.W[out][slot2] = o;
-        }
-      } else
-      for (unsigned q = gtid; q < nw; q += gthreads) {
-        const unsigned i = r == 1u ? q : __ldcg(&a.W[in][q]);
-        int x, y, z; x_coords(a, __ldcg(&a.deps[i]), x, y, z);
-        unsigned kc;
-        const uint32_t res = x_reseed_eval(a, i, x, y, z, kc);
-        const uint32_t was = __ldcg(&a.nc[i]);
-        a.nk[i] = (uint8_t)kc;
-        if (res == was) continue;
-        a.nc[i] = res;
-#pragma unroll
-        for (int k0 = 0; k0 < 24; k0 += XRC) {
-          unsigned o[XRC], so[XRC], ko[XRC];
-#pragma unroll
-          for (int t = 0; t < XRC; ++t) {
-            const int k = k0 + t, nx = x + x_dc(k, 0), ny = y + x_dc(k, 1), nz = z + x_dc(k, 2);
-            o[t] = x_in_grid(g, nx, ny, nz) ? __ldcg(&a.ord[x_vi(g, nx, ny, nz)]) : XNONE;
-          }
-#pragma unroll
-          for (int t = 0; t < XRC; ++t) so[t] = (o[t] != XNONE && o[t] > i) ? __ldcg(&a.wstamp[o[t]]) : wclock;
-#pragma unroll
-          for (int t = 0; t < XRC; ++t) ko[t] = (so[t] != wclock && r > 1u && so[t] != wclock - 1u) ? __ldcg(&a.nk[o[t]]) : XNONE;
-          unsigned pm = 0;
-#pragma unroll
-          for (int t = 0; t < XRC; ++t) {
-            const unsigned kd = (unsigned)(k0 + t) ^ 1u;
-            bool push = so[t] != wclock;
-            if (push && ko[t] != XNONE) push = kd == ko[t] || (kd < ko[t] && res >= 2u);
-            if (push && atomicExch(&a.wstamp[o[t]], wclock) != wclock) pm |= 1u << t;
-          }
-          unsigned slot2 = x_warp_append_n(&ctl->nW[out], (unsigned)__popc(pm), lane);
-#pragma unroll
-          for (int t = 0; t < XRC; ++t) if ((pm >> t) & 1u) a.W[out][slot2++] = o[t];
-        }
-      }
-      x_gsync(&ctl->bar, bar_target);
-    }
-    X_LAP(12);
-    const unsigned per = (a.ndep + G - 1u) / G;
-    const unsigned lo = min(a.ndep, b * per), hi = min(a.ndep, lo + per);
-    unsigned mine = 0;
-    for (unsigned i = lo + tid; i < hi; i += XT) mine += __ldcg(&a.nc[i]) >= 2u ? 1u : 0u;
-    unsigned tot;
-    x_block_scan(sh, mine, lane, wid, tot);
-    if (tid == 0) ctl->partial[b] = tot;
-    if (gtid == 0) { ctl->nW[0] = ctl->nW[1] = ctl->nW[2] = 0; }
-    x_gsync(&ctl->bar, bar_target);
-    if (wid == 0) {
-      unsigned before = 0, all = 0;
-      for (unsigned k = lane; k < G; k += 32u) { const unsigned c = __ldcg(&ctl->partial[k]); all += c; if (k < b) before += c; }
-#pragma unroll
-      for (int o = 16; o > 0; o >>= 1) { before += __shfl_xor_sync(0xffffffffu, before, o); all += __shfl_xor_sync(0xffffffffu, all, o); }
-      if (lane == 0) { sh.base = before; sh.total = all; }
-    }
-    __syncthreads();
-    unsigned run = nE + sh.base;
-    for (unsigned i0 = lo; i0 < hi; i0 += XT) {
-      const unsigned i = i0 + tid;
-      uint32_t c = FB_INF, v = 0;
-      if (i < hi) {
-        c = __ldcg(&a.nc[i]); v = __ldcg(&a.deps[i]);
-        a.cobs[v] = c;
-        a.LS[v] = a.ls_deps + i;
-      }
-      unsigned ctot;
-      const unsigned pos = x_block_scan(sh, (i < hi && c >= 2u) ? 1u : 0u, lane, wid, ctot);
-      if (i < hi && c >= 2u) a.E[0][run + pos] = v;
-      run += ctot;
-    }
-    nE += sh.total;
-    x_gsync(&ctl->bar, bar_target);
-    X_LAP(13);
-  }
   bool big = nE > a.small_max;
 
   ++gen;
@@ -1003,7 +1052,7 @@
   }
   if (gtid == 0) {
     ctl->gen_id = gen; ctl->wclock = wclock; ctl->tclock = tclock; ctl->sclock = sclock;
-    ctl->generations = generations; ctl->reseed_rounds = reseed_rounds; ctl->rounds = rounds_total; ctl->dense_rounds = dense_total; ctl->voxels_changed = changed_total;
+    ctl->generations = generations; ctl->rounds = rounds_total; ctl->dense_rounds = dense_total; ctl->voxels_changed = changed_total;
   }
 }
 
@@ -1035,14 +1084,16 @@
   int per_sm = 0, sms = 0;
   for (const void *k : {(const void *)k_x_relax<false>, (const void *)k_x_relax<true>})
     if (cudaOccupancyMaxActiveBlocksPerMultiprocessor(&per_sm, k, XT, sizeof(XNb) * XW) != cudaSuccess || per_sm < 1) return -1;
+  for (const void *k : {(const void *)k_x_reseed<false>, (const void *)k_x_reseed<true>})
+    if (cudaOccupancyMaxActiveBlocksPerMultiprocessor(&per_sm, k, XT, 0) != cudaSuccess || per_sm < 1) return -1;
   if (cudaDeviceGetAttribute(&sms, cudaDevAttrMultiProcessorCount, device) != cudaSuccess) return -1;
   return sms;
 }
 
-cudaError_t fb_xrelax_launch(FbExact *X, const FbGeom &g, uint32_t *cobs, unsigned nE0, const uint32_t *deps, unsigned ndep, uint32_t *ord, uint32_t *nc, uint8_t *nk,
+cudaError_t fb_xrelax_launch(FbExact *X, const FbGeom &g, uint32_t *cobs, const uint32_t *deps, unsigned ndep, uint32_t *ord, uint32_t *nc, uint32_t *M,
                              const uint32_t *occbits, unsigned long long ls_deps, unsigned long long *dbg, cudaStream_t s) {
   XArgs a;
-  a.deps = deps; a.ndep = ndep; a.ord = ord; a.nc = nc; a.nk = nk; a.occbits = occbits; a.ls_deps = ls_deps;
+  a.deps = deps; a.ndep = ndep; a.ord = ord; a.nc = nc; a.M = M; a.occbits = occbits; a.ls_deps = ls_deps;
   fb_div_make((unsigned)g.pz, a.div_pz_m, a.div_pz_s);
   fb_div_make((unsigned)g.gy, a.div_gy_m, a.div_gy_s);
   a.g = g;
@@ -1051,9 +1102,13 @@
   a.cobs = cobs; a.MB = X->MB; a.LS = X->LS; a.SUM = X->SUM; a.SUMg = X->SUMg;
   a.E[0] = X->E[0]; a.E[1] = X->E[1]; a.emask = X->emask;
   for (int k = 0; k < 3; ++k) { a.W[k] = X->W[k]; a.F[k] = X->F[k]; }
-  a.wstamp = X->wstamp; a.slotc = X->slotc; a.ctl = X->d_ctl; a.nE0 = nE0; a.small_max = X->small_max; a.dense_min = X->dense_min; a.dbg = dbg;
+  a.wstamp = X->wstamp; a.slotc = X->slotc; a.ctl = X->d_ctl; a.small_max = X->small_max; a.dense_min = X->dense_min; a.dbg = dbg;
   a.async_on = X->async ? 1u : 0u;
   a.small_async_on = X->small_async ? 1u : 0u;
   void *args[] = {(void *)&a};
+  if (ndep) {
+    const cudaError_t e = cudaLaunchCooperativeKernel(dbg ? (void *)k_x_reseed<true> : (void *)k_x_reseed<false>, dim3(X->relax_blocks), dim3(XT), args, 0, s);
+    if (e != cudaSuccess) return e;
+  }
   return cudaLaunchCooperativeKernel(dbg ? (void *)k_x_relax<true> : (void *)k_x_relax<false>, dim3(X->relax_blocks), dim3(XT), args, sizeof(XNb) * XW, s);
 }
```
